# yhao-wang/DenseRetrievalToolkits

Hardware: AMD Instinct MI355X
Metric: queries/sec@top-1000, 10Mx768 corpus (BASELINE: passages encoded/sec + queries/sec@top-1000, 10Mx768 corpus, 1/2/4/8 GPU) (higher is better)
Workload: dtype bf16

## Files before the change

denseretrievaltoolkits_amd/_native.py:

```python
from __future__ import annotations

import ctypes
import os
import threading

import torch

from .build_native import LIB_PATH

DRT_OK = 0
DRT_EINVAL = -1
ROW_STATS_LEN = 34

_lock = threading.Lock()
_lib = None

c_i32 = ctypes.c_int32
c_i64 = ctypes.c_int64
c_sz = ctypes.c_size_t
c_vp = ctypes.c_void_p
c_f32 = ctypes.c_float
c_u64 = ctypes.c_uint64

_SIGNATURES = [
    ("drt_version", ctypes.c_char_p, []),
    ("drt_ip_topk_workspace", c_sz, [c_i64, c_i64, c_i32, c_i32]),
    ("drt_ip_topk_bf16", c_i32, [c_vp, c_i64, c_vp, c_i64, c_i32, c_i32, c_i64, c_vp, c_vp, c_vp, c_vp, c_sz, c_vp]),
    ("drt_ip_topk_resolve_workspace", c_sz, [c_i64, c_i64, c_i32]),
    ("drt_ip_topk_resolve", c_i32, [c_vp, c_i64, c_vp, c_i64, c_i32, c_i32, c_i64, c_vp, c_vp, c_vp, c_vp, c_sz,
                                    c_vp, c_vp]),
    ("drt_topk_merge", c_i32, [c_vp, c_vp, c_i64, c_i32, c_i32, c_i32, c_vp, c_vp, c_vp]),
    ("drt_ip_topk_sample_rank", c_i32, [c_i32]),
    ("drt_ip_topk_dist_workspace", c_sz, [c_i64, c_i64, c_i64, c_i32, c_i32]),
    ("drt_ip_topk_dist_sample", c_i32, [c_vp, c_i64, c_vp, c_i64, c_i64, c_i32, c_i32, c_vp, c_vp, c_sz, c_vp]),
    ("drt_ip_topk_dist_tau", c_i32, [c_vp, c_i64, c_i32, c_i32, c_vp, c_vp]),
    ("drt_ip_topk_dist_filter", c_i32, [c_vp, c_i64, c_vp, c_i64, c_i64, c_i32, c_i32, c_i64, c_vp, c_vp, c_vp,
                                        c_sz, c_vp]),
    ("drt_ip_topk_dist_filter_chunks", c_i32, [c_vp, c_i64, c_vp, c_i64, c_i64, c_i32, c_i32, c_i64, c_vp, c_vp,
                                               c_vp, c_i32, c_vp, c_sz, c_vp]),
    ("drt_ip_topk_tighten_rank", c_i32, [c_i64, c_i32, c_i32]),
    ("drt_ip_topk_filter_passes_workspace", c_sz, [c_i64, c_i64, c_i64, c_i32, c_i32]),
    ("drt_ip_topk_filter_passes", c_i32, [c_vp, c_i64, c_vp, c_i64, c_i64, c_i32, c_i32, c_i64, c_vp, c_vp,
                                          c_i32, c_i32, c_vp, c_vp, c_vp, c_sz, c_vp]),
    ("drt_ip_topk_dist_filter_lists", c_i32, [c_vp, c_i64, c_vp, c_i64, c_i64, c_i32, c_i32, c_i64, c_vp, c_i32,
                                              c_vp, c_vp, c_vp, c_sz, c_vp]),
    ("drt_ip_topk_dist_filter_lists_at", c_i32, [c_vp, c_i64, c_vp, c_i64, c_i64, c_i32, c_i32, c_i64, c_vp,
                                                 c_i32, c_i64, c_vp, c_vp, c_vp, c_sz, c_vp]),
    ("drt_topk_merge_packed", c_i32, [c_vp, c_i64, c_i32, c_i32, c_i64, c_vp, c_vp, c_vp, c_vp]),
    ("drt_topk_merge_packed_cert", c_i32, [c_vp, c_i64, c_i32, c_i32, c_i32, c_i64, c_vp, c_vp, c_vp, c_vp]),
    ("drt_topk_merge_packed_capped", c_i32, [c_vp, c_i64, c_i32, c_i32, c_i32, c_i32, c_i64, c_vp, c_vp, c_vp,
                                             c_vp]),
    ("drt_row_stats_bf16", c_i32, [c_vp, c_i64, c_i32, c_vp, c_i32, c_vp]),
    ("drt_refine_width", c_i32, [c_i32]),
    ("drt_ip_topk_exact_bf16", c_i32, [c_vp, c_i64, c_vp, c_i64, c_i32, c_i32, c_i64, c_vp, c_vp, c_vp, c_vp, c_vp,
                                       c_sz, c_vp]),
    ("drt_hit_metrics_i8", c_i32, [c_vp, c_i64, c_i64, c_vp, c_i32, c_vp, c_vp]),
    ("drt_answer_match_i32", c_i32, [c_vp, c_i32, c_vp, c_vp, c_i64, c_i64, c_i64, c_vp, c_vp, c_i32, c_i32, c_vp,
                                     c_vp, c_vp]),
    ("drt_ip_topk_resolve_exact", c_i32, [c_vp, c_i64, c_vp, c_i64, c_i32, c_i32, c_i64, c_vp, c_vp, c_vp, c_vp,
                                          c_vp, c_sz, c_vp, c_vp]),
    ("drt_ip_topk_resolve_wide_workspace", c_sz, [c_i64, c_i32]),
    ("drt_ip_topk_resolve_wide", c_i32, [c_vp, c_i64, c_vp, c_i64, c_i32, c_i32, c_i64, c_vp, c_vp, c_vp, c_vp,
                                         c_vp, c_sz, c_vp, c_vp]),
    ("drt_ip_topk_large_workspace", c_sz, [c_i32, c_i32]),
    ("drt_ip_topk_large", c_i32, [c_vp, c_i64, c_vp, c_i64, c_i32, c_i32, c_i64, c_vp, c_vp, c_vp, c_vp, c_vp, c_vp,
                                  c_sz, c_vp]),
    ("drt_ip_topk_large_keys", c_i32, [c_vp, c_i64, c_vp, c_i64, c_i32, c_i32, c_i64, c_vp, c_vp, c_vp, c_vp, c_vp,
                                       c_vp, c_vp, c_sz, c_vp]),
    ("drt_merge_exact", c_i32, [c_vp, c_vp, c_i64, c_i32, c_i32, c_vp, c_vp, c_vp]),
    ("drt_refine_delta_bf16", c_i32, [c_vp, c_i64, c_i32, c_vp, c_i64, c_i64, c_vp, c_vp, c_i32, c_i32, c_vp, c_vp,
                                      c_vp, c_vp, c_vp, c_vp]),
    ("drt_refine_delta_local_bf16", c_i32, [c_vp, c_i64, c_i32, c_vp, c_i64, c_i64, c_vp, c_vp, c_i32, c_i32, c_vp,
                                            c_vp, c_vp, c_vp, c_vp, c_vp]),
    ("drt_refine_sort", c_i32, [c_vp, c_vp, c_vp, c_vp, c_i64, c_i32, c_i32, c_vp, c_vp, c_vp]),
    ("drt_topk_exclude", c_i32, [c_vp, c_vp, c_i64, c_i32, c_vp, c_vp, c_vp, c_i32, c_i32, c_vp, c_vp, c_vp, c_vp]),
    ("drt_pair_scores_bf16", c_i32, [c_vp, c_i64, c_vp, c_i64, c_i32, c_vp, c_vp, c_i64, c_vp, c_vp]),
    ("drt_gemm_nt_bf16_f32", c_i32, [c_vp, c_vp, c_vp, c_i64, c_i64, c_i32, c_i64, c_vp]),
    ("drt_embed_ln", c_i32, [c_vp, c_vp, c_i64, c_i64, c_vp, c_vp, c_vp, c_vp, c_vp, c_f32, c_i32, c_vp, c_vp]),
    ("drt_linear_bf16", c_i32, [c_vp, c_vp, c_vp, c_vp, c_vp, c_i64, c_i64, c_i64, c_i32, c_vp]),
    ("drt_linear_workspace", c_sz, [c_i64, c_i64, c_i64]),
    ("drt_linear_bf16_ws", c_i32, [c_vp, c_vp, c_vp, c_vp, c_vp, c_i64, c_i64, c_i64, c_i32, c_vp, c_sz, c_vp]),
    ("drt_linear_ln_bf16_ws", c_i32, [c_vp, c_vp, c_vp, c_vp, c_vp, c_vp, c_f32, c_vp, c_vp, c_i64, c_i64, c_i64,
                                      c_vp, c_sz, c_vp]),
    ("drt_layernorm_f32_bf16", c_i32, [c_vp, c_i64, c_i32, c_vp, c_vp, c_f32, c_vp, c_vp]),
    ("drt_attention_fwd_lse_bf16", c_i32, [c_vp, c_vp, c_vp, c_vp, c_i64, c_i64, c_i32, c_i32, c_f32, c_vp]),
    ("drt_layernorm_bwd_workspace", c_sz, [c_i64, c_i32]),
    ("drt_layernorm_bwd_drop_bf16", c_i32, [c_vp, c_vp, c_vp, c_f32, c_i64, c_i32, c_vp, c_vp, c_vp, c_f32, c_u64,
                                            c_u64, c_vp, c_vp, c_vp, c_sz, c_vp]),
    ("drt_layernorm_bwd_sum_bf16", c_i32, [c_vp, c_vp, c_vp, c_f32, c_i64, c_i32, c_vp, c_vp, c_vp, c_f32, c_u64,
                                           c_u64, c_vp, c_vp, c_vp, c_vp, c_sz, c_vp]),
    ("drt_linear_bf16_ex", c_i32, [c_vp, c_vp, c_vp, c_vp, c_vp, c_vp, c_vp, c_i64, c_i64, c_i64, c_i32, c_f32, c_u64,
                                   c_u64, c_vp, c_sz, c_vp]),
    ("drt_layernorm_bwd_bf16", c_i32, [c_vp, c_vp, c_vp, c_f32, c_i64, c_i32, c_vp, c_vp, c_vp, c_vp, c_vp, c_sz,
                                       c_vp]),
    ("drt_colsum_workspace", c_sz, [c_i64, c_i64]),
    ("drt_colsum_bf16", c_i32, [c_vp, c_i64, c_i64, c_vp, c_vp, c_sz, c_vp]),
    ("drt_colsum_f32", c_i32, [c_vp, c_i64, c_i64, c_vp, c_vp, c_sz, c_vp]),
    ("drt_linear_dgelu_bias_workspace", c_sz, [c_i64, c_i64, c_i64]),
    ("drt_linear_dgelu_bias_bf16", c_i32, [c_vp, c_vp, c_vp, c_vp, c_i64, c_i64, c_i64, c_vp, c_vp, c_sz, c_vp]),
    ("drt_gelu_bwd_bf16", c_i32, [c_vp, c_vp, c_i64, c_vp, c_vp]),
    ("drt_linear_wgrad_workspace", c_sz, [c_i64, c_i64, c_i64]),
    ("drt_linear_wgrad_bf16", c_i32, [c_vp, c_vp, c_vp, c_i64, c_i64, c_i64, c_vp, c_sz, c_vp]),
    ("drt_transpose_bf16", c_i32, [c_vp, c_i64, c_i64, c_vp, c_vp]),
    ("drt_transpose_bf16_ld", c_i32, [c_vp, c_i64, c_i64, c_vp, c_i64, c_vp]),
    ("drt_embed_ln_pre", c_i32, [c_vp, c_vp, c_i64, c_i64, c_vp, c_vp, c_vp, c_vp, c_vp, c_f32, c_i32, c_vp, c_vp,
                                 c_vp]),
    ("drt_gelu_bf16", c_i32, [c_vp, c_i64, c_vp, c_vp]),
    ("drt_embedding_bwd", c_i32, [c_vp, c_vp, c_vp, c_i64, c_i64, c_i32, c_i64, c_vp, c_vp, c_vp, c_vp]),
    ("drt_embedding_bwd_types", c_i32, [c_vp, c_vp, c_i32, c_vp, c_i64, c_i64, c_i32, c_i64, c_vp, c_vp, c_vp,
                                         c_vp]),
    ("drt_attention_train_fwd_bf16", c_i32, [c_vp, c_vp, c_vp, c_vp, c_i64, c_i64, c_i32, c_i32, c_f32, c_f32,
                                             ctypes.c_uint64, ctypes.c_uint64, c_vp]),
    ("drt_attention_train_bwd_bf16", c_i32, [c_vp, c_vp, c_vp, c_vp, c_vp, c_vp, c_i64, c_i64, c_i32, c_i32, c_f32,
                                             c_f32, ctypes.c_uint64, ctypes.c_uint64, c_vp]),
    ("drt_dropout_add_bf16", c_i32, [c_vp, c_vp, c_i64, c_f32, ctypes.c_uint64, ctypes.c_uint64, c_vp, c_vp]),
    ("drt_attention_train_fwd_bits_bf16", c_i32, [c_vp, c_vp, c_vp, c_vp, c_vp, c_i64, c_i64, c_i32, c_i32, c_f32,
                                                  c_f32, c_u64, c_u64, c_vp]),
    ("drt_attention_train_bwd_bits_bf16", c_i32, [c_vp, c_vp, c_vp, c_vp, c_vp, c_vp, c_vp, c_i64, c_i64, c_i32,
                                                  c_i32, c_f32, c_f32, c_u64, c_u64, c_vp]),
    ("drt_attention_train_bwd_bias_workspace", c_sz, [c_i64, c_i32, c_i32]),
    ("drt_attention_train_bwd_bias_bf16", c_i32, [c_vp, c_vp, c_vp, c_vp, c_vp, c_vp, c_vp, c_i64, c_i64, c_i32,
                                                  c_i32, c_f32, c_f32, c_u64, c_u64, c_vp, c_vp, c_sz, c_vp]),
    ("drt_attention_bwd_bf16", c_i32, [c_vp, c_vp, c_vp, c_vp, c_vp, c_vp, c_i64, c_i64, c_i32, c_i32, c_f32, c_vp]),
    ("drt_layernorm_bf16", c_i32, [c_vp, c_i64, c_i32, c_vp, c_vp, c_f32, c_vp, c_vp]),
    ("drt_attention_bf16", c_i32, [c_vp, c_vp, c_vp, c_i64, c_i64, c_i32, c_i32, c_f32, c_vp]),
    ("drt_pool_bf16", c_i32, [c_vp, c_vp, c_i64, c_i64, c_i32, c_i32, c_vp, c_vp, c_vp]),
# ... 62 lines not shown
```

denseretrievaltoolkits_amd/csrc/search.hip:

```cpp
#include <cmath>

#include "profile.h"
#include "search_internal.h"

namespace drt {

constexpr int kHitCap = 1024;
constexpr int kTopRL = 4;

__host__ __device__ __forceinline__ int pass_tiles(int ntiles, int npass, int pass) {
  return npass <= 1 ? ntiles : (pass < ntiles ? (ntiles - 1 - pass) / npass + 1 : 0);
}

__device__ __forceinline__ void glds16(const void* gsrc, uint32_t lds_addr) {
  uint32_t keep;
  asm volatile(
      "s_mov_b32 %0, m0\n\t"
      "s_mov_b32 m0, %2\n\t"
      "s_nop 0\n\t"
      "global_load_lds_dwordx4 %1, off\n\t"
      "s_mov_b32 m0, %0"
      : "=&s"(keep)
      : "v"(gsrc), "s"(lds_addr)
      : "memory");
}

__device__ __forceinline__ void glds16_nt(const void* gsrc, uint32_t lds_addr) {
  uint32_t keep;
  asm volatile(
      "s_mov_b32 %0, m0\n\t"
      "s_mov_b32 m0, %2\n\t"
      "s_nop 0\n\t"
      "global_load_lds_dwordx4 %1, off nt\n\t"
      "s_mov_b32 m0, %0"
      : "=&s"(keep)
      : "v"(gsrc), "s"(lds_addr)
      : "memory");
}

__device__ __forceinline__ uint32_t lds_addr_of(const void* p) {
  return (uint32_t)(uintptr_t)(const __attribute__((address_space(3))) char*)p;
}

template <int N>
__device__ __forceinline__ void wait_vmcnt() {
  asm volatile("s_waitcnt vmcnt(%0)" ::"n"(N) : "memory");
}

__device__ __forceinline__ void lds_barrier() {
  asm volatile("s_waitcnt lgkmcnt(0)" ::: "memory");
  __builtin_amdgcn_s_barrier();
}

__device__ __forceinline__ void push_hit(const ScanArgs& a, int q_local,
                                         int64_t q, uint64_t key, uint32_t* hit_n,
                                         uint64_t* hk, uint16_t* hq) {
  const uint32_t p = atomicAdd(hit_n, 1u);
  if (p < (uint32_t)kHitCap) {
    hk[p] = key;
    hq[p] = (uint16_t)q_local;
  } else {
    const uint32_t g = atomicAdd(a.counts + q * kCntStride, 1u);
    if (g < (uint64_t)a.cap) ((uint64_t*)a.out)[q * a.cap + g] = key;
  }
}

template <int NT>
__device__ __forceinline__ void flush_hits_agg(const ScanArgs& a, int64_t qbase, uint32_t n, const uint64_t* hk,
                                               const uint16_t* hq, uint32_t* qcnt, uint32_t* qoff) {
  n = n < (uint32_t)kHitCap ? n : (uint32_t)kHitCap;
  for (int i = threadIdx.x; i < kQueriesPerWG; i += NT) qcnt[i] = 0;
  lds_barrier();
  uint32_t rank[(kHitCap + NT - 1) / NT];
#pragma unroll
  for (int u = 0; u < (kHitCap + NT - 1) / NT; ++u) {
    const uint32_t i = threadIdx.x + u * NT;
    if (i < n) rank[u] = atomicAdd(&qcnt[hq[i]], 1u);
  }
  lds_barrier();
  for (int q = threadIdx.x; q < kQueriesPerWG; q += NT) {
    const uint32_t c = qcnt[q];
    qoff[q] = (c && qbase + q < a.nq) ? atomicAdd(a.counts + (qbase + q) * kCntStride, c) : 0u;
  }
  lds_barrier();
#pragma unroll
  for (int u = 0; u < (kHitCap + NT - 1) / NT; ++u) {
    const uint32_t i = threadIdx.x + u * NT;
    if (i < n) {
      const int ql = hq[i];
      const uint32_t g = qoff[ql] + rank[u];
      if (g < (uint64_t)a.cap) ((uint64_t*)a.out)[(qbase + ql) * a.cap + g] = hk[i];
    }
  }
}

// ... 314 lines not shown
  for (int64_t it = 0; it < my_tiles; ++it) {
    const int64_t tile = t0 + it * tstep;
    const int64_t younger = my_tiles - 1 - it;
    wait_tiles_younger<C::GLDS_PER_WAVE>((int)(younger < C::PD - 1 ? younger : C::PD - 1));
    lds_barrier();

    if (MODE == SCAN_FILTER) {
      const uint32_t n = *hit_n;
      if (n >= (uint32_t)(kHitCap / 2)) {
        if (AGG) flush_hits_agg<NW * 64>(a, qbase, n, hk, hq, qcnt, qoff);
        else flush_hits<NW * 64>(a, qbase, n, hk, hq);
        lds_barrier();
        if (tid == 0) *hit_n = 0;
        lds_barrier();
      }
    }
    if (it + C::PD < my_tiles)
      issue_tile16<D, NW>(a, ring + nslot * C::TILE_BYTES, tile + C::PD * tstep, wave, lane);

    const int64_t rowbase = tile * kT16 + 4 * kq;
    if ((it & 1) == 0) {
      mma_tile(accA, buf);
      if (it > 0) epilogue(accB, rbB);
      rbA = rowbase;
    } else {
      mma_tile(accB, buf);
      epilogue(accA, rbA);
      rbB = rowbase;
    }
    buf = (buf + 1 == C::NBUF) ? 0 : buf + 1;
    nslot = (nslot + 1 == C::NBUF) ? 0 : nslot + 1;
  }

  if (my_tiles & 1) epilogue(accA, rbA);
  else epilogue(accB, rbB);

  if (MODE == SCAN_TOPR) {
#pragma unroll
    for (int b = 0; b < QB; ++b) {
      if (!qok[b]) continue;
      uint32_t* o = (uint32_t*)a.out + qg[b] * a.cap + ((int64_t)blockIdx.x * 4 + kq) * kTopRL;
#pragma unroll
      for (int i = 0; i < kTopRL; ++i) o[i] = topl[b][i];
    }
  }
  if (MODE == SCAN_FILTER) {
    lds_barrier();
    const uint32_t nf = *hit_n;
    if (AGG) flush_hits_agg<NW * 64>(a, qbase, nf, hk, hq, qcnt, qoff);
    else flush_hits<NW * 64>(a, qbase, nf, hk, hq);
  }
}

constexpr int kWaveSeg = kHitCap / 8;

__device__ __forceinline__ void wave_flush_hits(const ScanArgs& a, int64_t qw, const uint64_t* hk,
                                                const uint8_t* hq, int n, int lane) {
  for (int i = lane; i < n; i += 64) {
    const uint64_t key = hk[i];
    const int64_t q = qw + hq[i];
    const uint32_t g = atomicAdd(a.counts + q * kCntStride, 1u);
    if (g < (uint64_t)a.cap) ((uint64_t*)a.out)[q * a.cap + g] = key;
  }
}

template <int D, bool NT = true>
__global__ __launch_bounds__(512, 1) void ip_scan16r_kernel(ScanArgs a) {
  constexpr int NW = 8;
  using C = Scan16Cfg<D, NW>;
  constexpr int PD = C::NBUF;
  __shared__ __attribute__((aligned(16))) char smem[C::LDS_BYTES];

  const int tid = threadIdx.x;
  const int wave = __builtin_amdgcn_readfirstlane(tid >> 6);
  const int lane = tid & 63;
  const int r = lane & 15;
  const int kq = lane >> 4;
  uint64_t* hk = (uint64_t*)(smem + C::HIT_KEY_OFF) + wave * kWaveSeg;
  uint8_t* hq = (uint8_t*)(smem + C::HIT_Q_OFF) + wave * kWaveSeg;

  const int64_t qbase = (int64_t)blockIdx.y * kQueriesPerWG;
  const int tmul = a.npass > 1 ? a.npass : 1;
  const int tph = a.npass > 1 ? a.pass : 0;
  const int tall = (int)((a.nrows + kT16 - 1) / kT16);
  const int ntiles = pass_tiles(tall, a.npass, a.pass);
  const uint32_t nrows = (uint32_t)a.nrows;
  const int t0 = blockIdx.x;
  const int tstep = gridDim.x;
  const int my_tiles = t0 < ntiles ? (ntiles - 1 - t0) / tstep + 1 : 0;
  if (my_tiles == 0) return;
  const int partial_tile = ((a.nrows & (kT16 - 1)) != 0 && (tall - 1) % tmul == tph) ? ntiles - 1 : -1;
  const uint32_t ring = lds_addr_of(smem);
  const int64_t tile_stride = (int64_t)tstep * tmul * kT16 * a.ldp * 2;
  const char* next_base = (const char*)(a.P + ((int64_t)t0 * tmul + tph) * kT16 * a.ldp);

  const int64_t qw = qbase + wave * 16;
  const int64_t qg = qw + r;
  const bool qok = qg < a.nq;
  const int64_t qs = qok ? qg : 0;
  bf16x8 qf[C::KS];
#pragma unroll
  for (int s = 0; s < C::KS; ++s) qf[s] = *(const bf16x8*)(a.Q + qs * a.ldq + s * 32 + kq * 8);
  float tau = __builtin_nanf("");
  {
    const float tv = a.tau[qs];
    tau = qok ? tv : tau;
  }
  if (!qok) {
#pragma unroll
    for (int s = 0; s < C::KS; ++s) qf[s] = (bf16x8){};
  }
#pragma unroll
  for (int s = 0; s < C::KS; ++s) asm volatile("" ::"v"(qf[s]));
  asm volatile("" ::"v"(tau));
  asm volatile("s_waitcnt vmcnt(0)" ::: "memory");

  LeanTile<D, NW> lt;
  lt.init(a, wave, lane);
#pragma unroll
  for (int p = 0; p < PD; ++p) {
    if (p < my_tiles) {
      const int tile = t0 + p * tstep;
      lt.template issue<NT>(a, ring + p * C::TILE_BYTES, next_base, tile == partial_tile, tile * tmul + tph, wave,
                            lane);
      next_base += tile_stride;
    }
  }
  if (wave >= NW / 2) __builtin_amdgcn_s_setprio(1);
  {
    const int last = my_tiles - 1 < PD - 1 ? my_tiles - 1 : PD - 1;
    wait_tiles_younger<C::GLDS_PER_WAVE>((int)last);
  }
  lds_barrier();

  const int sw = (r >> 1) & 7;
  int aoff[2];
#pragma unroll
  for (int m = 0; m < 2; ++m) aoff[m] = r * 128 + (((4 * m + kq) ^ sw) << 4);
  bf16x8 af[C::KS];
#pragma unroll
  for (int s = 0; s < C::KS; ++s) af[s] = *(const bf16x8*)(smem + (s >> 1) * (kT16 * 128) + aoff[s & 1]);

  auto mma_roll = [&](f32x4& acc, int nslot) {
    const char* nb = smem + nslot * C::TILE_BYTES;
    acc = (f32x4){0.f, 0.f, 0.f, 0.f};
#pragma unroll
    for (int s = 0; s < C::KS; ++s) {
      acc = __builtin_amdgcn_mfma_f32_16x16x32_bf16(af[s], qf[s], acc, 0, 0, 0);
      af[s] = *(const bf16x8*)(nb + (s >> 1) * (kT16 * 128) + aoff[s & 1]);
      __builtin_amdgcn_sched_barrier(0);
    }
  };
  int wcnt = 0;
  auto epilogue = [&](const f32x4& acc, uint32_t rowbase) {
    const float mx = fmaxf(fmaxf(acc[0], acc[1]), fmaxf(acc[2], acc[3])) - tau;
    if (__ballot(mx >= 0.0f) == 0ull) return;
    bool hv[4];
    uint64_t mv[4];
    int cv[4];
#pragma unroll
    for (int j = 0; j < 4; ++j) {
      hv[j] = acc[j] >= tau && rowbase + j < nrows;
      mv[j] = __ballot(hv[j]);
      cv[j] = __builtin_popcountll(mv[j]);
    }
    const int tot = cv[0] + cv[1] + cv[2] + cv[3];
    if (wcnt + tot <= kWaveSeg) {
      int base = wcnt;
#pragma unroll
      for (int j = 0; j < 4; ++j) {
        if (hv[j]) {
          const int pos = base + (int)__builtin_amdgcn_mbcnt_hi((uint32_t)(mv[j] >> 32),
                                                                __builtin_amdgcn_mbcnt_lo((uint32_t)mv[j], 0u));
          hk[pos] = ((uint64_t)desc_key(acc[j]) << 32) | (uint64_t)(a.row_base + rowbase + j);
          hq[pos] = (uint8_t)r;
        }
        base += cv[j];
      }
      wcnt = base;
      return;
    }
#pragma unroll
    for (int j = 0; j < 4; ++j) {
      const bool hit = acc[j] >= tau && rowbase + j < nrows;
      const uint64_t m = __ballot(hit);
      if (m == 0ull) continue;
      const int c = __builtin_popcountll(m);
      if (wcnt + c > kWaveSeg) {
        wave_flush_hits(a, qw, hk, hq, wcnt, lane);
        wcnt = 0;
      }
      if (hit) {
        const int pos = wcnt + (int)__builtin_amdgcn_mbcnt_hi((uint32_t)(m >> 32),
                                                              __builtin_amdgcn_mbcnt_lo((uint32_t)m, 0u));
        hk[pos] = ((uint64_t)desc_key(acc[j]) << 32) | (uint64_t)(a.row_base + rowbase + j);
        hq[pos] = (uint8_t)r;
      }
      wcnt += c;
    }
  };

  f32x4 accA, accB;
  uint32_t rbA = 0, rbB = 0;
  int buf = 0;
  auto iter = [&](int it, f32x4& acc, uint32_t& rb, const f32x4& prev, uint32_t rb_prev) {
    const int tile = t0 + it * tstep;
    if (it + PD <= my_tiles) {
      wait_vmcnt<C::GLDS_PER_WAVE * (PD - 2)>();
    } else if (it + 1 < my_tiles) {
      wait_tiles_younger<C::GLDS_PER_WAVE>(my_tiles - 1 - it - 1);
    }
    lds_barrier();
    if (it + PD < my_tiles) {
      const int ntile = tile + PD * tstep;
      lt.template issue<NT>(a, ring + buf * C::TILE_BYTES, next_base, ntile == partial_tile, ntile * tmul + tph,
                            wave, lane);
      next_base += tile_stride;
    }
    const int nslot = buf + 1 == C::NBUF ? 0 : buf + 1;
    mma_roll(acc, nslot);
    if (it > 0) epilogue(prev, rb_prev);
    rb = (uint32_t)(tile * tmul + tph) * kT16 + 4 * kq;
    buf = nslot;
  };
  for (int it = 0; it < my_tiles; it += 2) {
    iter(it, accA, rbA, accB, rbB);
    if (it + 1 < my_tiles) iter(it + 1, accB, rbB, accA, rbA);
  }
  if (my_tiles & 1) epilogue(accA, rbA);
  else epilogue(accB, rbB);
  if (wcnt) wave_flush_hits(a, qw, hk, hq, wcnt, lane);
}

template <int D>
struct Scan32Cfg {
  static constexpr int KS = D / 32;
  static constexpr int RD = KS % 2 == 0 ? 2 : 1;
  static constexpr int TILE_BYTES = kT16 * D * 2;
  static constexpr int HIT_BYTES = kHitCap * 9;
  static constexpr int NB_RAW = (160 * 1024 - HIT_BYTES) / TILE_BYTES;
  static constexpr int NB = NB_RAW > 6 ? 6 : NB_RAW;
  static constexpr int RING_BYTES = NB * TILE_BYTES;
  static constexpr int LDS_BYTES = RING_BYTES + HIT_BYTES;
  static_assert(NB >= 3, "ring too small");
  static_assert(LDS_BYTES <= 160 * 1024, "LDS budget");
};
constexpr int kQueriesPerWG32 = 256;

template <int D>
__global__ __launch_bounds__(512, 1) void ip_scan32r_kernel(ScanArgs a) {
  constexpr int NW = 8;
  using C = Scan16Cfg<D, NW>;
  using C32 = Scan32Cfg<D>;
  constexpr int NB = C32::NB;
  constexpr int PD = NB - 1;
  constexpr int KS = C32::KS;
  constexpr int RD = C32::RD;
  constexpr int kSeg = kHitCap / NW;
  __shared__ __attribute__((aligned(16))) char smem[C32::LDS_BYTES];

  const int tid = threadIdx.x;
  const int wave = __builtin_amdgcn_readfirstlane(tid >> 6);
  const int lane = tid & 63;
  const int r = lane & 15;
  const int kq = lane >> 4;
  uint64_t* hk = (uint64_t*)(smem + C32::RING_BYTES) + wave * kSeg;
  uint8_t* hq = (uint8_t*)(smem + C32::RING_BYTES + kHitCap * 8) + wave * kSeg;

  const int64_t qbase = (int64_t)blockIdx.y * kQueriesPerWG32;
  const int tmul = a.npass > 1 ? a.npass : 1;
  const int tph = a.npass > 1 ? a.pass : 0;
  const int tall = (int)((a.nrows + kT16 - 1) / kT16);
  const int ntiles = pass_tiles(tall, a.npass, a.pass);
  const uint32_t nrows = (uint32_t)a.nrows;
  const int t0 = blockIdx.x;
  const int tstep = gridDim.x;
  const int my_tiles = t0 < ntiles ? (ntiles - 1 - t0) / tstep + 1 : 0;
  if (my_tiles == 0) return;
  const int partial_tile = ((a.nrows & (kT16 - 1)) != 0 && (tall - 1) % tmul == tph) ? ntiles - 1 : -1;
  const uint32_t ring = lds_addr_of(smem);
  const int64_t tile_stride = (int64_t)tstep * tmul * kT16 * a.ldp * 2;
  const char* next_base = (const char*)(a.P + ((int64_t)t0 * tmul + tph) * kT16 * a.ldp);

  const int64_t qw = qbase + wave * 32;
  bf16x8 qf0[KS], qf1[KS];
  float tau0, tau1;
  {
    const int64_t g0 = qw + r, g1 = qw + 16 + r;
    const bool ok0 = g0 < a.nq, ok1 = g1 < a.nq;
    const int64_t s0 = ok0 ? g0 : 0, s1 = ok1 ? g1 : 0;
#pragma unroll
    for (int s = 0; s < KS; ++s) {
      qf0[s] = *(const bf16x8*)(a.Q + s0 * a.ldq + s * 32 + kq * 8);
      qf1[s] = *(const bf16x8*)(a.Q + s1 * a.ldq + s * 32 + kq * 8);
    }
    const float v0 = a.tau[s0], v1 = a.tau[s1];
    tau0 = ok0 ? v0 : __builtin_nanf("");
    tau1 = ok1 ? v1 : __builtin_nanf("");
    if (!ok0) {
#pragma unroll
      for (int s = 0; s < KS; ++s) qf0[s] = (bf16x8){};
    }
    if (!ok1) {
#pragma unroll
      for (int s = 0; s < KS; ++s) qf1[s] = (bf16x8){};
    }
  }
#pragma unroll
  for (int s = 0; s < KS; ++s) asm volatile("" ::"v"(qf0[s]), "v"(qf1[s]));
  asm volatile("" ::"v"(tau0), "v"(tau1));
  asm volatile("s_waitcnt vmcnt(0)" ::: "memory");

  LeanTile<D, NW> lt;
  lt.init(a, wave, lane);
#pragma unroll
  for (int p = 0; p < PD; ++p) {
    if (p < my_tiles) {
      const int tile = t0 + p * tstep;
      lt.template issue<false>(a, ring + p * C::TILE_BYTES, next_base, tile == partial_tile, tile * tmul + tph, wave,
                               lane);
      next_base += tile_stride;
    }
  }
  if (wave >= NW / 2) __builtin_amdgcn_s_setprio(1);
  {
    const int last = my_tiles - 1 < PD - 1 ? my_tiles - 1 : PD - 1;
    wait_tiles_younger<C::GLDS_PER_WAVE>((int)last);
  }
  lds_barrier();

  const int sw = (r >> 1) & 7;
  int aoff[2];
#pragma unroll
  for (int m = 0; m < 2; ++m) aoff[m] = r * 128 + (((4 * m + kq) ^ sw) << 4);
  auto frag = [&](int slot, int s) -> bf16x8 {
    return *(const bf16x8*)(smem + slot * C::TILE_BYTES + (s >> 1) * (kT16 * 128) + aoff[s & 1]);
  };
  bf16x8 af[RD];
#pragma unroll
  for (int s = 0; s < RD; ++s) af[s] = frag(0, s);

  int wcnt = 0;
  auto append = [&](const f32x4& acc, float tau, int ql, uint32_t rowbase) {
    const float mx = fmaxf(fmaxf(acc[0], acc[1]), fmaxf(acc[2], acc[3])) - tau;
    if (__ballot(mx >= 0.0f) == 0ull) return;
#pragma unroll
    for (int j = 0; j < 4; ++j) {
      const bool hit = acc[j] >= tau && rowbase + j < nrows;
      const uint64_t m = __ballot(hit);
      if (m == 0ull) continue;
      const int c = __builtin_popcountll(m);
      if (wcnt + c > kSeg) {
        wave_flush_hits(a, qw, hk, hq, wcnt, lane);
        wcnt = 0;
      }
      if (hit) {
        const int pos = wcnt + (int)__builtin_amdgcn_mbcnt_hi((uint32_t)(m >> 32),
                                                              __builtin_amdgcn_mbcnt_lo((uint32_t)m, 0u));
        hk[pos] = ((uint64_t)desc_key(acc[j]) << 32) | (uint64_t)(a.row_base + rowbase + j);
        hq[pos] = (uint8_t)ql;
      }
      wcnt += c;
    }
  };

  auto epilogue = [&](const f32x4& p0, const f32x4& p1, uint32_t rowbase) {
    append(p0, tau0, r, rowbase);
    append(p1, tau1, 16 + r, rowbase);
  };

  int buf = 0;
  auto iter = [&](int it, f32x4& acc0, f32x4& acc1, uint32_t& rb, const f32x4& prev0, const f32x4& prev1,
                  uint32_t rb_prev) {
    const int tile = t0 + it * tstep;
    if (it + PD <= my_tiles) {
      wait_vmcnt<C::GLDS_PER_WAVE * (PD - 2)>();
    } else if (it + 1 < my_tiles) {
      wait_tiles_younger<C::GLDS_PER_WAVE>(my_tiles - 1 - it - 1);
    }
    lds_barrier();
    const bool do_dma = it + PD < my_tiles;
    const int ntile = tile + PD * tstep;
    const int pslot = buf == 0 ? NB - 1 : buf - 1;
    const int nslot = buf + 1 == NB ? 0 : buf + 1;
    acc0 = (f32x4){0.f, 0.f, 0.f, 0.f};
    acc1 = (f32x4){0.f, 0.f, 0.f, 0.f};
#pragma unroll
    for (int s = 0; s < KS; ++s) {
      acc0 = __builtin_amdgcn_mfma_f32_16x16x32_bf16(af[s % RD], qf0[s], acc0, 0, 0, 0);
      acc1 = __builtin_amdgcn_mfma_f32_16x16x32_bf16(af[s % RD], qf1[s], acc1, 0, 0, 0);
      af[s % RD] = s + RD < KS ? frag(buf, s + RD) : frag(nslot, s + RD - KS);
      __builtin_amdgcn_sched_barrier(0);
      if (s == KS / 4 && do_dma) {
        lt.template issue<false>(a, ring + pslot * C::TILE_BYTES, next_base, ntile == partial_tile,
                                 ntile * tmul + tph, wave, lane);
        next_base += tile_stride;
      }
      __builtin_amdgcn_sched_barrier(0);
    }
    if (it > 0) epilogue(prev0, prev1, rb_prev);
    rb = (uint32_t)(tile * tmul + tph) * kT16 + 4 * kq;
    buf = nslot;
  };
  f32x4 a0, a1, b0, b1;
  uint32_t rbA = 0, rbB = 0;
  for (int it = 0; it < my_tiles; it += 2) {
    iter(it, a0, a1, rbA, b0, b1, rbB);
    if (it + 1 < my_tiles) iter(it + 1, b0, b1, rbB, a0, a1, rbA);
  }
  if (my_tiles & 1) epilogue(a0, a1, rbA);
  else epilogue(b0, b1, rbB);
  if (wcnt) wave_flush_hits(a, qw, hk, hq, wcnt, lane);
}

struct TopkPlan : PlanHead {
  int64_t n, k, nq, nq_pad;
  bool sample;
  int64_t cap;
  int64_t m;
  int64_t stride;
  int64_t r;
  int64_t nchunk;
  int64_t kc;
  size_t off_cs, off_ci, off_delta, off_rcnt, total;
};

static size_t plan_refine_tail(TopkPlan& p) {
  p.kc = refine_width(p.k);
  WsBump b{p.head_end};
  p.off_cs = b.take((size_t)p.nq_pad * p.kc * 4);
  p.off_ci = b.take((size_t)p.nq_pad * p.kc * 8);
  p.off_delta = b.take((size_t)p.nq_pad * p.kc * 4);
  p.off_rcnt = b.take((size_t)p.nq_pad * 8);
  return b.o;
}

static double poisson_tail_ge(double lam, int64_t r) {
  double logp = -lam + r * std::log(lam) - std::lgamma((double)r + 1.0);
  double p = std::exp(logp), s = 0.0;
  for (int64_t i = r; i < r + 2000; ++i) {
    s += p;
    p *= lam / (double)(i + 1);
    if (p < 1e-30 * s) break;
  }
  return s;
}


static TopkPlan make_plan(int64_t nq, int64_t n, int64_t k) {
  TopkPlan p{};
  p.n = n;
  p.k = k;
  p.nq = nq;
  p.nq_pad = (nq + kQueriesPerWG - 1) / kQueriesPerWG * kQueriesPerWG;
  const int64_t target = hit_target(k);
  p.cap = 4 * target;
  if (n <= p.cap) {
    p.sample = false;
    p.cap = align_up(std::max<int64_t>(n, 4), 4);
    p.m = 0;
    p.stride = 1;
    p.r = 0;
  } else {
    p.sample = true;
    int64_t r = 1;
    while (poisson_tail_ge((double)k * r / (double)target, r) > 1e-9 && r < 100000) ++r;
    p.r = r;
    int64_t m = (r * n + target - 1) / target;
    if (m > n) m = n;
    p.stride = std::max<int64_t>(1, n / m);
    const int64_t m_cap = std::max<int64_t>(1, kKthChunk / r) * kKthChunk;
    if (m > m_cap) m = m_cap;
    p.stride = std::max<int64_t>(1, n / m);
    p.m = (n - p.stride / 2 + p.stride - 1) / p.stride;
    if (p.m > m_cap) p.m = m_cap;
    if (p.m < r) p.m = std::min<int64_t>(n, r);
    p.nchunk = (p.m + kKthChunk - 1) / kKthChunk;
  }
  static_cast<PlanHead&>(p) = plan_head_layout(p.nq_pad, p.cap, p.sample ? 8 : 4, p.m, p.nchunk * p.r);
  p.total = plan_refine_tail(p);
  return p;
}

static TopkPlan make_dist_plan(int64_t nq, int64_t n_local, int64_t n_global, int64_t k) {
  const TopkPlan g = make_plan(nq, n_global, k);
  TopkPlan p{};
  p.n = n_local;
  p.k = k;
  p.nq = nq;
  p.nq_pad = g.nq_pad;
  const int64_t target = hit_target(k);
  p.cap = std::max<int64_t>(g.cap, 4 * target);
  p.sample = g.sample;
  p.r = g.sample ? g.r : 0;
  p.stride = 1;
  p.m = 0;
  p.nchunk = 0;
  if (p.sample && n_local > 0) {
    int64_t m = (p.r * n_local + target - 1) / target;
    if (m > n_local) m = n_local;
    const int64_t m_cap = std::max<int64_t>(1, kKthChunk / p.r) * kKthChunk;
    if (m > m_cap) m = m_cap;
    p.stride = std::max<int64_t>(1, n_local / m);
    p.m = (n_local - p.stride / 2 + p.stride - 1) / p.stride;
    if (p.m > m_cap) p.m = m_cap;
    p.nchunk = (p.m + kKthChunk - 1) / kKthChunk;
  }
  static_cast<PlanHead&>(p) = plan_head_layout(p.nq_pad, p.cap, 8, p.m, p.nchunk * p.r);
  p.total = p.head_end;
  return p;
}

static int64_t rows_exp_hits(const TopkPlan& p, int64_t rows, int64_t n_global) {
  return p.sample ? std::max<int64_t>(1, hit_target(p.k) * rows / std::max<int64_t>(1, n_global)) : rows;
}

static int64_t pass_exp_hits(const TopkPlan& p, int64_t npasses, int64_t n_global) {
  return p.sample ? std::max<int64_t>(1, hit_target(p.k) * p.n / npasses / std::max<int64_t>(1, n_global))
                  : std::max<int64_t>(1, p.n / npasses);
}

static int scan_grid_x(int64_t ntiles) {
  int dev = 0, cus = 256;
  if (hipGetDevice(&dev) == hipSuccess) {
    int v = 0;
    if (hipDeviceGetAttribute(&v, hipDeviceAttributeMultiprocessorCount, dev) == hipSuccess && v > 0)
      cus = v;
  }
  const int64_t g = std::min<int64_t>(ntiles, (int64_t)cus);
  return (int)std::max<int64_t>(g, 1);
}

static dim3 scan16_grid(int64_t nq, int64_t nrows, int qpw = kQueriesPerWG) {
  const unsigned gy = (unsigned)((nq + qpw - 1) / qpw);
  const int64_t ntiles = (nrows + kT16 - 1) / kT16;
  int gx = scan_grid_x(ntiles);
  if (gy > 1 && ntiles >= 8) {
    const int cus = scan_grid_x((int64_t)1 << 40);
    const int share = std::max(8, (cus / (int)gy) & ~7);
    gx = (int)std::min<int64_t>(ntiles, share);
  }
  return dim3(gx, gy);
}

template <int D>
static int launch_scan_d(const ScanArgs& a, int mode, hipStream_t s) {
  if (a.nq == 0 || a.nrows == 0) return DRT_OK;
  constexpr bool kLean = D <= 768;
  if (a.npass > 1 && (mode != SCAN_FILTER || !kLean || a.row0 != 0 || a.rstride != 1 || a.pass < 0 ||
                      a.pass >= a.npass))
    return DRT_EINVAL;
  const int64_t ntiles = pass_tiles((int)((a.nrows + kT16 - 1) / kT16), a.npass, a.pass);
  if (ntiles == 0) return DRT_OK;
  const dim3 grid = scan16_grid(a.nq, ntiles * kT16);
  const unsigned gy = grid.y;
  if (mode == SCAN_FILTER) {
    const double eh = a.exp_hits > 0 ? (double)a.exp_hits : (double)a.cap / 4.0;
    const bool dense_hits = eh * 256.0 / (double)a.nrows >= 0.35;
    bool lean = false;
    if constexpr (kLean) {
      lean = a.row0 == 0 && a.rstride == 1;
      if (lean) {
        if (gy > 1) {
          const dim3 grid32 = scan16_grid(a.nq, ntiles * kT16, kQueriesPerWG32);
          hipLaunchKernelGGL((ip_scan32r_kernel<D>), grid32, dim3(512), 0, s, a);
        } else {
          hipLaunchKernelGGL((ip_scan16r_kernel<D, true>), grid, dim3(512), 0, s, a);
        }
      }
    }
    if (!lean) {
      if (dense_hits) hipLaunchKernelGGL((ip_scan16_kernel<D, SCAN_FILTER, 8, true>), grid, dim3(512), 0, s, a);
      else hipLaunchKernelGGL((ip_scan16_kernel<D, SCAN_FILTER, 8, false>), grid, dim3(512), 0, s, a);
    }
  } else if (mode == SCAN_TOPR) {
    hipLaunchKernelGGL((ip_scan16_kernel<D, SCAN_TOPR>), grid, dim3(512), 0, s, a);
  } else {
    hipLaunchKernelGGL((ip_scan16_kernel<D, SCAN_DENSE>), grid, dim3(512), 0, s, a);
  }
  return hip_status(hipGetLastError());
}

static int launch_scan_impl(const ScanArgs& a, int d, int mode, hipStream_t s) {
  switch (d) {
    case 64: return launch_scan_d<64>(a, mode, s);
    case 128: return launch_scan_d<128>(a, mode, s);
    case 192: return launch_scan_d<192>(a, mode, s);
    case 256: return launch_scan_d<256>(a, mode, s);
    case 320: return launch_scan_d<320>(a, mode, s);
    case 384: return launch_scan_d<384>(a, mode, s);
    case 448: return launch_scan_d<448>(a, mode, s);
    case 512: return launch_scan_d<512>(a, mode, s);
    case 576: return launch_scan_d<576>(a, mode, s);
    case 640: return launch_scan_d<640>(a, mode, s);
    case 704: return launch_scan_d<704>(a, mode, s);
    case 768: return launch_scan_d<768>(a, mode, s);
    case 832: return launch_scan_d<832>(a, mode, s);
    case 896: return launch_scan_d<896>(a, mode, s);
    case 960: return launch_scan_d<960>(a, mode, s);
    case 1024: return launch_scan_d<1024>(a, mode, s);
    default: return DRT_EINVAL;
  }
}

int launch_scan(const ScanArgs& a, int d, int mode, hipStream_t s, int family) {
  const ProfPair pp = prof_begin(family, s);
  const int rc = launch_scan_impl(a, d, mode, s);
  prof_end(pp, s);
  return rc;
}

static bool valid_dist_dims(int64_t nq, int64_t n_local, int64_t n_global, int32_t d, int32_t k) {
  return nq >= 0 && n_local >= 0 && n_global >= n_local && d > 0 && d % 64 == 0 && d <= 1024 && k >= 1 &&
         k <= kSelMaxK && n_global < (int64_t)0xFFFFFFFFll;
}

}

using namespace drt;

extern "C" {

const char* drt_version(void) {
  return "drt-mi355x 0.3 (gfx950; packed top-k lists: entry k = valid count << 32 | flags)";
}

size_t drt_ip_topk_workspace(int64_t nq, int64_t n, int32_t d, int32_t k) {
  if (!valid_dims(nq, n, d, k)) return 0;
  return make_plan(nq, n, k).total;
}

static int ip_topk_impl(const void* Q, int64_t nq, const void* P, int64_t n, int32_t d, int32_t k,
                        int64_t id_offset, float* out_scores, int64_t* out_ids, int32_t* status, void* ws,
                        size_t ws_bytes, const float* stats, hipStream_t s) {
  DRT_REQUIRE(valid_dims(nq, n, d, k));
  if (nq == 0) return DRT_OK;
  DRT_REQUIRE(Q && out_scores && out_ids && ws);
  const TopkPlan p = make_plan(nq, n, k);
  DRT_REQUIRE(ws_bytes >= p.total);
  char* w = (char*)ws;
  float* tau = (float*)(w + p.off_tau);
  uint32_t* cnt = (uint32_t*)(w + p.off_cnt);
  const bool refine = stats != nullptr && n > 0;

  SelectArgs sa{};
  sa.k = k;
  sa.nq = nq;
// ... 291 lines not shown
};

static int filter_setup(FilterRun& f, const void* Q, int64_t nq, const void* P, int64_t n_local, int64_t n_global,
                        int32_t d, int32_t k, int64_t id_offset, const void* thr, uint64_t* packed, void* ws,
                        size_t ws_bytes, void* stream) {
  DRT_REQUIRE(valid_dist_dims(nq, n_local, n_global, d, k));
  DRT_REQUIRE(id_offset >= 0 && id_offset + n_local <= n_global);
  if (nq == 0) return DRT_OK;
  DRT_REQUIRE(Q && thr && packed && ws);
  f.p = make_dist_plan(nq, n_local, n_global, k);
  DRT_REQUIRE(ws_bytes >= f.p.total);
  f.s = (hipStream_t)stream;
  f.w = (char*)ws;
  f.cnt = (uint32_t*)(f.w + f.p.off_cnt);
  f.sel = SelectArgs{};
  f.sel.in = f.w + f.p.off_keys;
  f.sel.in_stride = f.p.cap;
  f.sel.k = k;
  f.sel.nq = nq;
  f.sel.id_offset = id_offset;
  f.sel.out_packed = packed;
  f.sel.global_tau = true;
  f.scan = filter_scan_args(Q, nq, P, d, n_local, nullptr, f.cnt, f.w + f.p.off_keys, f.p.cap);
  return DRT_OK;
}

static int filter_begin(const FilterRun& f, bool zero_counts) {
  DRT_REQUIRE(f.scan.P != nullptr);
  if (zero_counts) DRT_CHECK_HIP(hipMemsetAsync(f.cnt, 0, f.p.nq_pad * 4 * kCntStride, f.s));
  return DRT_OK;
}

static int filter_select(FilterRun& f) {
  if (f.p.n == 0) return launch_select(f.sel, SEL_DENSE32, SEL_TOPK, f.s);
  f.sel.counts = f.cnt;
  f.sel.cap = f.p.cap;
  f.sel.n_total = f.p.n;
  return launch_select(f.sel, SEL_KEYS64, SEL_TOPK, f.s);
}

int drt_ip_topk_dist_filter(const void* Q, int64_t nq, const void* P, int64_t n_local, int64_t n_global, int32_t d,
                            int32_t k, int64_t id_offset, const float* tau, uint64_t* packed, void* ws,
                            size_t ws_bytes, void* stream) {
  FilterRun f;
  int rc = filter_setup(f, Q, nq, P, n_local, n_global, d, k, id_offset, tau, packed, ws, ws_bytes, stream);
  if (rc || nq == 0) return rc;
  if (n_local > 0) {
    if ((rc = filter_begin(f, true))) return rc;
    ScanArgs a = f.scan;
    a.tau = tau;
    a.exp_hits = rows_exp_hits(f.p, n_local, n_global);
    if ((rc = launch_scan(a, d, SCAN_FILTER, f.s, PROF_SCAN))) return rc;
  }
  return filter_select(f);
}

int drt_ip_topk_dist_filter_chunks(const void* Q, int64_t nq, const void* P, int64_t n_local, int64_t n_global,
                                   int32_t d, int32_t k, int64_t id_offset, const float* tau, uint64_t* packed,
                                   const int64_t* starts, int32_t nchunks, void* ws, size_t ws_bytes, void* stream) {
  DRT_REQUIRE(d <= 768 && n_local < ((int64_t)1 << 32));
  DRT_REQUIRE(starts != nullptr && nchunks >= 1 && starts[0] == 0 && starts[nchunks] == n_local);
  for (int c = 0; c < nchunks; ++c) DRT_REQUIRE(starts[c] <= starts[c + 1]);
  FilterRun f;
  int rc = filter_setup(f, Q, nq, P, n_local, n_global, d, k, id_offset, tau, packed, ws, ws_bytes, stream);
  if (rc || nq == 0) return rc;
  if (n_local > 0) {
    if ((rc = filter_begin(f, true))) return rc;
    for (int c = 0; c < nchunks; ++c) {
      const int64_t r0 = starts[c], rows = starts[c + 1] - starts[c];
      if (rows == 0) continue;
      ScanArgs a = f.scan;
      a.P += r0 * d;
      a.nrows = rows;
      a.row_base = (uint32_t)r0;
      a.tau = tau;
      a.exp_hits = rows_exp_hits(f.p, rows, n_global);
      if ((rc = launch_scan(a, d, SCAN_FILTER, f.s, PROF_SCAN))) return rc;
    }
  }
  return filter_select(f);
}

int32_t drt_ip_topk_tighten_rank(int64_t n_local, int32_t npasses, int32_t k) {
  if (n_local <= 0 || npasses <= 1 || k < 1) return 0;
  const int64_t tall = (n_local + kT16 - 1) / kT16;
  const int64_t t0 = (tall + npasses - 1) / npasses;
  if (t0 >= tall) return 0;
  const double C = (double)tall / (double)t0;
  for (int64_t r = 1; r < ((int64_t)1 << 24); ++r) {
    const double sigma = std::sqrt(C * (C - 1.0) * (double)r + (C - 1.0) * (double)r);
    if (C * (double)r - 5.0 * sigma >= (double)k) return (int32_t)r;
  }
  return 0;
}

size_t drt_ip_topk_filter_passes_workspace(int64_t nq, int64_t n_local, int64_t n_global, int32_t d, int32_t k) {
  if (!valid_dist_dims(nq, n_local, n_global, d, k)) return 0;
  const TopkPlan p = make_dist_plan(nq, n_local, n_global, k);
  return passes_layout(p.total, p.nq_pad).total;
}

int drt_ip_topk_filter_passes(const void* Q, int64_t nq, const void* P, int64_t n_local, int64_t n_global,
                              int32_t d, int32_t k, int64_t id_offset, const float* tau, uint64_t* packed,
                              int32_t npasses, int32_t r, float* tau1_out, uint32_t* pass0_out, void* ws,
                              size_t ws_bytes, void* stream) {
  DRT_REQUIRE(d <= 768 && n_local < ((int64_t)1 << 32) && npasses >= 1 && npasses <= 1024);
  FilterRun f;
  int rc = filter_setup(f, Q, nq, P, n_local, n_global, d, k, id_offset, tau, packed, ws, ws_bytes, stream);
  if (rc || nq == 0) return rc;
  const PassesLayout pl = passes_layout(f.p.total, f.p.nq_pad);
  DRT_REQUIRE(ws_bytes >= pl.total);
  if (r < 0) r = drt_ip_topk_tighten_rank(n_local, npasses, k);
  const int tall = (int)((n_local + kT16 - 1) / kT16);
  const bool tighten = r > 0 && n_local > 0 && pass_tiles(tall, npasses, 0) < tall;
  if (!tighten) {
    if (tau1_out) DRT_CHECK_HIP(hipMemcpyAsync(tau1_out, tau, (size_t)nq * 4, hipMemcpyDeviceToDevice, f.s));
    if (pass0_out) DRT_CHECK_HIP(hipMemsetAsync(pass0_out, 0, (size_t)nq * 16, f.s));
  }
  float* tau1 = tau1_out ? tau1_out : (float*)(f.w + f.p.off_tau);
  uint32_t* pass0 = pass0_out ? pass0_out : (uint32_t*)(f.w + pl.off_pass0);
  if (n_local > 0) {
    if ((rc = filter_begin(f, true))) return rc;
    for (int ps = 0; ps < npasses; ++ps) {
      if (pass_tiles(tall, npasses, ps) == 0) continue;
      ScanArgs a = f.scan;
      a.npass = npasses;
      a.pass = ps;
      a.tau = (tighten && ps > 0) ? tau1 : tau;
      a.exp_hits = pass_exp_hits(f.p, npasses, n_global);
      if ((rc = launch_scan(a, d, SCAN_FILTER, f.s, PROF_SCAN))) return rc;
      if (tighten && ps == 0) {
        const ProfPair pp = prof_begin(PROF_SELECT, f.s);
        launch_tighten(nq, (const uint64_t*)f.scan.out, f.p.cap, f.cnt, tau, (int)r, tau1, pass0, f.s);
        prof_end(pp, f.s);
        DRT_CHECK_HIP(hipGetLastError());
      }
    }
  }
  f.sel.pass0 = tighten ? pass0 : nullptr;
  return filter_select(f);
}

int drt_ip_topk_dist_filter_lists(const void* Q, int64_t nq, const void* P, int64_t n_local, int64_t n_global,
                                  int32_t d, int32_t k, int64_t id_offset, const uint32_t* lists, int32_t nlists,
                                  float* tau_out, uint64_t* packed, void* ws, size_t ws_bytes, void* stream) {
  const int32_t r = drt_ip_topk_sample_rank(k);
  return drt_ip_topk_dist_filter_lists_at(Q, nq, P, n_local, n_global, d, k, id_offset, lists, nlists,
                                          r > 0 ? nq * r : 0, tau_out, packed, ws, ws_bytes, stream);
}

int drt_ip_topk_dist_filter_lists_at(const void* Q, int64_t nq, const void* P, int64_t n_local, int64_t n_global,
                                     int32_t d, int32_t k, int64_t id_offset, const uint32_t* lists, int32_t nlists,
                                     int64_t lists_stride, float* tau_out, uint64_t* packed, void* ws,
                                     size_t ws_bytes, void* stream) {
  const int32_t r = drt_ip_topk_sample_rank(k);
  DRT_REQUIRE(r > 0 && nlists >= 1 && (int64_t)nlists * r <= kKthChunk);
  DRT_REQUIRE(nlists == 1 || lists_stride >= nq * r);
  FilterRun f;
  int rc = filter_setup(f, Q, nq, P, n_local, n_global, d, k, id_offset, lists, packed, ws, ws_bytes, stream);
  if (rc || nq == 0) return rc;
  float* tau = tau_out ? tau_out : (float*)(f.w + f.p.off_tau);
  launch_kth_final(nq, lists, (int)nlists, (int)r, lists_stride, (int64_t)r, tau, nullptr,
                   n_local > 0 ? f.cnt : nullptr, (int)r, f.s);
  DRT_CHECK_HIP(hipGetLastError());
  if (n_local > 0) {
    if ((rc = filter_begin(f, false))) return rc;
    ScanArgs a = f.scan;
    a.tau = tau;
    a.exp_hits = rows_exp_hits(f.p, n_local, n_global);
    if ((rc = launch_scan(a, d, SCAN_FILTER, f.s, PROF_SCAN))) return rc;
  }
  return filter_select(f);
}

}
```

denseretrievaltoolkits_amd/csrc/search_internal.h:

```cpp
#pragma once

#include <algorithm>
#include <vector>

#include "drt_common.h"

#define DRT_INTERNAL __attribute__((visibility("hidden")))

namespace drt {

constexpr int kQueriesPerWG = 128;
constexpr int kCntStride = 32;
constexpr int kSelMaxK = 2048;
constexpr int kKthChunk = 4096;
constexpr int64_t kWideCap = 65536;

enum { SEL_KEYS64 = 0, SEL_DENSE32 = 1 };
enum { SEL_TOPK = 0, SEL_KTH = 1 };

struct SelectArgs {
  const void* in;
  int64_t in_stride;
  const uint32_t* counts;
  int64_t n_in;
  int64_t cap;
  int64_t n_total;
  int k;
  int64_t nq;
  float* out_scores;
  int64_t* out_ids;
  int64_t ldo;
  int64_t id_offset;
  int32_t* status;
  const int32_t* qmap;
  float* tau;
  uint64_t* out_packed;
  bool global_tau;
  int k_cert;
  const uint32_t* pass0;
};

DRT_INTERNAL int launch_select(const SelectArgs& a, int input, int output, hipStream_t s);
DRT_INTERNAL bool kth_rank_fits(int64_t m, int64_t r);
DRT_INTERNAL void launch_kth_rank(int64_t nq, const uint32_t* in, int64_t stride, int64_t n, int r, float* tau,
                                  uint32_t* zero, hipStream_t s);
DRT_INTERNAL void launch_kth_partial(int64_t nchunk, int64_t nq, const uint32_t* in, int64_t stride, int64_t n, int r,
                                     uint32_t* part, hipStream_t s);
DRT_INTERNAL void launch_kth_final(int64_t nq, const uint32_t* part, int nlists, int r, int64_t lstride,
                                   int64_t qstride, float* tau, uint32_t* best, uint32_t* zero, int len,
                                   hipStream_t s);
DRT_INTERNAL void launch_tighten(int64_t nq, const uint64_t* keys, int64_t cap, const uint32_t* counts,
                                 const float* tau0, int r, float* tau1, uint32_t* pass0, hipStream_t s);

enum { SCAN_FILTER = 0, SCAN_DENSE = 1, SCAN_TOPR = 2 };

struct ScanArgs {
  const __bf16* Q;
  int64_t nq;
  int64_t ldq;
  const __bf16* P;
  int64_t ldp;
  int64_t row0;
  int64_t nrows;
  int64_t rstride;
  const float* tau;
  uint32_t* counts;
  void* out;
  int64_t cap;
  int64_t exp_hits;
  uint32_t row_base;
  int32_t npass;
  int32_t pass;
};

static inline ScanArgs scan_args(const void* Q, int64_t nq, const void* P, int32_t d) {
  ScanArgs a{};
  a.Q = (const __bf16*)Q;
  a.nq = nq;
  a.ldq = d;
  a.P = (const __bf16*)P;
  a.ldp = d;
  a.row0 = 0;
  a.rstride = 1;
  return a;
}

static inline ScanArgs filter_scan_args(const void* Q, int64_t nq, const void* P, int32_t d, int64_t n,
                                        const float* tau, uint32_t* counts, void* out, int64_t cap) {
  ScanArgs a = scan_args(Q, nq, P, d);
  a.nrows = n;
  a.tau = tau;
  a.counts = counts;
  a.out = out;
  a.cap = cap;
  return a;
}

DRT_INTERNAL int launch_scan(const ScanArgs& a, int d, int mode, hipStream_t s, int family);

struct RefineArgs {
  const __bf16* Q;
  int64_t nq;
  int32_t d;
  const __bf16* P;
  int64_t n_local;
  int64_t row_offset;
  const float* cs;
  const int64_t* ci;
  int32_t kc, k;
  const float* stats;
  const float* tau;
  float* delta;
  int32_t* cnt;
  int32_t* status;
  const int32_t* qmap;
  bool set_status;
  int32_t slice;
  float* out_s;
  int64_t* out_i;
};

DRT_INTERNAL int launch_refine(RefineArgs& ra, hipStream_t s);
DRT_INTERNAL int flagged_queries(const int32_t* status, int64_t nq, int32_t mask, int32_t want, hipStream_t s,
                                 std::vector<int32_t>& out);
DRT_INTERNAL int gather_queries(const void* Q, int32_t d, const int32_t* idx, int64_t nb, void* qbuf, void* qmap,
                                hipStream_t s);

static inline size_t align_up(size_t x, size_t a) { return (x + a - 1) / a * a; }

static inline int64_t hit_target(int64_t k) { return std::max<int64_t>(4096, 4 * k); }

static inline int64_t refine_width(int64_t k) {
  return std::min<int64_t>(kSelMaxK, k + std::max<int64_t>(256, k / 4));
}

static inline bool valid_dims(int64_t nq, int64_t n, int32_t d, int32_t k) {
  return nq >= 0 && n >= 0 && d > 0 && d % 64 == 0 && d <= 1024 && k >= 1 && k <= kSelMaxK &&
         n < (int64_t)0xFFFFFFFFll;
}


struct WsBump {
  size_t o = 0;
  size_t take(size_t bytes) {
    const size_t at = o;
    o = align_up(o + bytes, 256);
    return at;
  }
};

struct PlanHead {
  size_t off_tau, off_cnt, off_keys, off_sample, off_part, head_end;
};
static inline PlanHead plan_head_layout(int64_t nq_pad, int64_t cap, int key_bytes, int64_t m, int64_t part_keys) {
  WsBump b;
  PlanHead h;
  h.off_tau = b.take((size_t)nq_pad * 4);
  h.off_cnt = b.take((size_t)nq_pad * 4 * kCntStride);
  h.off_keys = b.take((size_t)nq_pad * cap * key_bytes);
  h.off_sample = b.take((size_t)nq_pad * align_up(m, 4) * 4);
  h.off_part = b.take((size_t)nq_pad * part_keys * 4);
  h.head_end = b.o;
  return h;
}

struct PassesLayout {
  size_t off_pass0, total;
};
static inline PassesLayout passes_layout(size_t plan_total, int64_t nq_pad) {
  WsBump b;
  b.take(plan_total);
  PassesLayout l;
  l.off_pass0 = b.take((size_t)nq_pad * 16);
  l.total = b.o;
  return l;
}

static inline int64_t resolve_width(int64_t n) { return align_up(std::max<int64_t>(n, 4), 4); }

struct ResolveLayout {
  size_t qbuf, scores, qmap, cand_s, cand_i, delta, cnt, total;
};
static inline ResolveLayout resolve_layout(int64_t chunk, int64_t n, int32_t d, int64_t kc = kSelMaxK) {
  WsBump b;
  ResolveLayout l;
  l.qbuf = b.take((size_t)chunk * d * 2);
  l.scores = b.take((size_t)chunk * resolve_width(n) * 4);
  l.qmap = b.take((size_t)chunk * 4);
  l.cand_s = b.take((size_t)chunk * kSelMaxK * 16 + chunk * 8);
  l.cand_i = l.cand_s + (size_t)chunk * kc * 4;
  l.delta = l.cand_s + (size_t)chunk * kc * 12;
  l.cnt = l.cand_s + (size_t)chunk * kc * 16;
  l.total = b.o;
  return l;
}

struct WideLayout {
  size_t qbuf, qmap, tau, counts, keys, ekeys, total;
};
static inline WideLayout wide_layout(int32_t d) {
  const size_t B = kQueriesPerWG;
  WsBump b;
  WideLayout l;
  l.qbuf = b.take(B * d * 2);
  l.qmap = b.take(B * 4);
  l.tau = b.take(B * 4);
  l.counts = b.take(B * kCntStride * 4);
  l.keys = b.take(B * kWideCap * 8);
  l.ekeys = b.take(B * kWideCap * 8);
  l.total = b.o;
  return l;
}

struct LargeLayout {
  WideLayout wide;
  size_t sel_k, sel_r, sel_n, bin_k, bin_r, total;
};
static inline LargeLayout large_layout(int32_t d, int32_t k) {
  const size_t B = kQueriesPerWG;
  LargeLayout l;
  l.wide = wide_layout(d);
  WsBump b{l.wide.total};
  l.sel_k = b.take(B * k * 8);
  l.sel_r = b.take(B * k * 4);
  l.sel_n = b.take(B * 4);
  l.bin_k = b.take(B * k * 8);
  l.bin_r = b.take(B * k * 4);
  l.total = b.o;
  return l;
}

}
```

denseretrievaltoolkits_amd/csrc/select.hip:

```cpp
#include "profile.h"
#include "search_internal.h"

namespace drt {

constexpr int kSelThreads = 512;
constexpr int kSelWaves = kSelThreads / 64;
constexpr int kSelBins = 1024;
constexpr int kSelBuf = 4096;
constexpr int kSelKPT = 16;
constexpr int kSelRegCap = kSelKPT * kSelThreads;

template <int INPUT>
__device__ __forceinline__ uint64_t sel_load(const SelectArgs& a, int64_t q, int64_t j) {
  if (INPUT == SEL_KEYS64) return ((const uint64_t*)a.in)[q * a.in_stride + j];
  const uint32_t v = ((const uint32_t*)a.in)[q * a.in_stride + j];
  return ((uint64_t)v << 32) | (uint64_t)(uint32_t)j;
}

__device__ __forceinline__ float key_score(uint64_t x) { return desc_key_to_score((uint32_t)(x >> 32)); }

__device__ __forceinline__ int score_bin(float s, float smin, float scale) {
  if (scale == 0.0f) return 0;
  return hist_bin((s - smin) * scale, kSelBins, __builtin_signbit(s) ? 0 : kSelBins - 1);
}
// ... 376 lines not shown
              cnt = bb[t];
              break;
            }
            run += bb[t];
          }
          const int64_t rem = kk - run;
          sh_prefix = prefix | ((uint64_t)d << shift);
          sh_mask = mask | (255ull << shift);
          sh_kk = rem;
          if ((int64_t)cnt == rem) sh_done = 1;
        }
      }
      __syncthreads();
    }
    const uint64_t thr = sh_prefix | ~sh_mask;
    if (tid == 0) sh_nsel = 0;
    __syncthreads();
    for (int64_t j = tid; j < c; j += kSelThreads) {
      const uint64_t x = sel_load<INPUT>(a, q, j);
      if (x <= thr) {
        const uint32_t p = atomicAdd(&sh_nsel, 1u);
        if (p < (uint32_t)kSelBuf) buf[p] = x;
      }
    }
    __syncthreads();
    nsel = (int)sh_nsel;
  }

  nsel = nsel < kSelBuf ? nsel : kSelBuf;
  int n2 = 1;
  while (n2 < nsel) n2 <<= 1;
  for (int i = nsel + tid; i < n2; i += kSelThreads) buf[i] = ~0ull;
  __syncthreads();
  block_bitonic(buf, n2);

  const int64_t orow = a.qmap ? (int64_t)a.qmap[q] : q;
  if (a.out_packed) {
    uint64_t* op = a.out_packed + orow * (int64_t)(a.k + 1);
    for (int j = tid; j < a.k; j += kSelThreads) {
      if (j < kk_total) {
        const uint64_t x = buf[j];
        op[j] = (x & 0xFFFFFFFF00000000ull) | (uint64_t)(uint32_t)(a.id_offset + (int64_t)(x & 0xFFFFFFFFull));
      } else {
        op[j] = ~0ull;
      }
    }
    if (tid == 0) {
      const uint64_t nval = (uint64_t)(kk_total < a.k ? kk_total : a.k);
      bool bad = INPUT == SEL_KEYS64 && c_raw > a.cap;
      if (INPUT == SEL_KEYS64 && a.pass0) {
        const uint32_t* t = a.pass0 + q * 4;
        if (t[2] && (int64_t)t[1] + (c_raw - (int64_t)t[0]) < (int64_t)a.k) bad = true;
      }
      op[a.k] = (nval << 32) | (bad ? 1ull : 0ull) | (c_raw > (int64_t)a.k ? 2ull : 0ull);
    }
    return;
  }
  float* os = a.out_scores + orow * a.ldo;
  int64_t* oi = a.out_ids + orow * a.ldo;
  for (int j = tid; j < a.k; j += kSelThreads) {
    if (j < kk_total) {
      const uint64_t x = buf[j];
      os[j] = key_score(x);
      oi[j] = a.id_offset + (int64_t)(x & 0xFFFFFFFFull);
    } else {
      os[j] = kPadScore;
      oi[j] = -1;
    }
  }
  if (a.status && tid == 0) {
    int st = 0;
    if (INPUT == SEL_KEYS64) {
      if (c_raw > a.cap) st = 1;
      const int64_t kq = a.k_cert > 0 ? a.k_cert : a.k;
      if (!a.global_tau && c_raw < kq && c_raw < a.n_total) st = 1;
    }
    a.status[orow] = st;
  }
}

constexpr int kTightThreads = 256;

__global__ __launch_bounds__(kTightThreads) void tighten_kernel(const uint64_t* keys, int64_t cap,
                                                                const uint32_t* counts, const float* tau0, int r,
                                                                float* tau1, uint32_t* pass0) {
  __shared__ uint32_t hist[256];
  __shared__ uint32_t sh_prefix, sh_rem;
  __shared__ uint32_t red[kTightThreads / 64];
  const int tid = threadIdx.x;
  const int64_t q = blockIdx.x;
  const uint32_t c = counts[q * kCntStride];
  const float t0 = tau0[q];
  if (!((int64_t)c <= cap && c >= (uint32_t)r && t0 == t0)) {
    if (tid == 0) {
      tau1[q] = t0;
      pass0[q * 4 + 0] = c;
      pass0[q * 4 + 1] = c;
      pass0[q * 4 + 2] = 0;
      pass0[q * 4 + 3] = 0;
    }
    return;
  }
  const uint64_t* kq = keys + q * cap;
  uint32_t prefix = 0, mask = 0, rem = (uint32_t)r;
  for (int shift = 24; shift >= 0; shift -= 8) {
    hist[tid] = 0;
    __syncthreads();
    for (uint32_t j = tid; j < c; j += kTightThreads) {
      const uint32_t key = (uint32_t)(kq[j] >> 32);
      if ((key & mask) == prefix) atomicAdd(&hist[(key >> shift) & 255], 1u);
    }
    __syncthreads();
    if (tid < 64) {
      const uint32_t bb[4] = {hist[4 * tid], hist[4 * tid + 1], hist[4 * tid + 2], hist[4 * tid + 3]};
      const uint32_t s4 = bb[0] + bb[1] + bb[2] + bb[3];
      uint32_t incl = s4;
#pragma unroll
      for (int o = 1; o < 64; o <<= 1) {
        const uint32_t v = __shfl_up(incl, o, 64);
        if (tid >= o) incl += v;
      }
      uint32_t run = incl - s4;
      if (run < rem && rem <= incl) {
        int dgt = 4 * tid;
#pragma unroll
        for (int t = 0; t < 3; ++t) {
          if (dgt == 4 * tid + t && run + bb[t] < rem) {
            run += bb[t];
            ++dgt;
          }
        }
        sh_prefix = prefix | ((uint32_t)dgt << shift);
        sh_rem = rem - run;
      }
    }
    __syncthreads();
    prefix = sh_prefix;
    rem = sh_rem;
    mask |= 255u << shift;
  }
  const float t1 = desc_key_to_score(prefix);
  uint32_t n = 0;
  for (uint32_t j = tid; j < c; j += kTightThreads) n += key_score(kq[j]) >= t1 ? 1u : 0u;
#pragma unroll
  for (int o = 32; o > 0; o >>= 1) n += __shfl_xor(n, o, 64);
  if ((tid & 63) == 0) red[tid >> 6] = n;
  __syncthreads();
  if (tid == 0) {
    uint32_t tot = 0;
    for (int w = 0; w < kTightThreads / 64; ++w) tot += red[w];
    tau1[q] = t1;
    pass0[q * 4 + 0] = c;
    pass0[q * 4 + 1] = tot;
    pass0[q * 4 + 2] = t1 > t0 ? 1u : 0u;
    pass0[q * 4 + 3] = 0;
  }
}

constexpr int kKthThreads = 512;

__device__ __forceinline__ void block_bitonic_u32(uint32_t* buf, int n2) { block_sort<uint32_t, kKthThreads>(buf, n2); }

constexpr int kKthPer = kKthChunk / kKthThreads;
constexpr int kKthBins = 256;
constexpr int kKthSel = 1024;

__global__ __launch_bounds__(kKthThreads) void kth_partial_kernel(const uint32_t* in, int64_t stride, int64_t n,
                                                                  int r, uint32_t* part) {
  __shared__ __attribute__((aligned(16))) uint32_t buf[kKthChunk];
  __shared__ uint32_t hist[kKthThreads / 64][kKthBins];
  __shared__ float red[2][kKthThreads / 64];
  __shared__ uint32_t sh_n;
  __shared__ int sh_bin;
  const int tid = threadIdx.x, wave = tid >> 6, lane = tid & 63;
  const int64_t q = blockIdx.y;
  const int nchunk = gridDim.x;
  const int64_t j0 = (int64_t)blockIdx.x * kKthChunk;
  const int cnt = (int)(n - j0 < kKthChunk ? n - j0 : kKthChunk);
  const uint32_t* src = in + q * stride + j0;

  uint32_t key[kKthPer];
#pragma unroll
  for (int v = 0; v < 2; ++v) {
    const int base = v * (kKthChunk / 2) + 4 * tid;
    if (base + 3 < cnt) {
      const u32x4 x = *(const u32x4*)(src + base);
#pragma unroll
      for (int u = 0; u < 4; ++u) key[4 * v + u] = x[u];
    } else {
#pragma unroll
      for (int u = 0; u < 4; ++u) key[4 * v + u] = base + u < cnt ? src[base + u] : 0xFFFFFFFFu;
    }
  }
  float hi = -__builtin_inff(), lo = __builtin_inff();
#pragma unroll
  for (int e = 0; e < kKthPer; ++e) {
    if (key[e] != 0xFFFFFFFFu) {
      const float sc = desc_key_to_score(key[e]);
      hi = fmaxf(hi, sc);
      lo = fminf(lo, sc);
    }
  }
#pragma unroll
  for (int o = 32; o > 0; o >>= 1) {
    hi = fmaxf(hi, __shfl_xor(hi, o, 64));
    lo = fminf(lo, __shfl_xor(lo, o, 64));
  }
  if (lane == 0) {
    red[0][wave] = hi;
    red[1][wave] = lo;
  }
  for (int i = tid; i < (kKthThreads / 64) * kKthBins; i += kKthThreads) (&hist[0][0])[i] = 0;
  __syncthreads();
#pragma unroll
  for (int w = 0; w < kKthThreads / 64; ++w) {
    hi = fmaxf(hi, red[0][w]);
    lo = fminf(lo, red[1][w]);
  }
  const float range = hi - lo;
  const float scale = hist_scale((float)kKthBins, range);
  int bins[kKthPer];
#pragma unroll
  for (int e = 0; e < kKthPer; ++e) {
    int bb = kKthBins;
    if (key[e] != 0xFFFFFFFFu) {
      const float sc = desc_key_to_score(key[e]);
      bb = scale == 0.0f ? 0 : hist_bin((hi - sc) * scale, kKthBins, __builtin_signbit(sc) ? kKthBins - 1 : 0);
      atomicAdd(&hist[wave][bb], 1u);
    }
    bins[e] = bb;
  }
  __syncthreads();
  if (tid < 64) {
    uint32_t c4[4];
    uint32_t s4 = 0;
#pragma unroll
    for (int t = 0; t < 4; ++t) {
// ... 197 lines not shown
  if (nsel <= kRankBuf) {
    int n2 = 1;
    while (n2 < nsel) n2 <<= 1;
    for (int i = nsel + tid; i < n2; i += kRankThreads) buf[i] = kPad;
    __syncthreads();
    block_sort<uint32_t, kRankThreads>(buf, n2);
    kth = r <= nsel ? buf[r - 1] : kPad;
  } else {
    if (tid == 0) {
      sh_rem = (uint32_t)r;
      sh_prefix = 0;
    }
    uint32_t mask = 0;
    for (int shift = 24; shift >= 0; shift -= 8) {
      if (tid < 256) hist[tid] = 0;
      __syncthreads();
      const uint32_t prefix = sh_prefix;
#pragma unroll
      for (int e = 0; e < kRankPer; ++e)
        if (key[e] <= T && (key[e] & mask) == prefix)
          atomicAdd(&hist[(key[e] >> shift) & 255u], 1u);
      __syncthreads();
      if (tid == 0) {
        uint32_t rem = sh_rem, dgt = 255;
        for (uint32_t dd = 0; dd < 256; ++dd) {
          if (hist[dd] >= rem) {
            dgt = dd;
            break;
          }
          rem -= hist[dd];
        }
        sh_rem = rem;
        sh_prefix = prefix | (dgt << shift);
      }
      mask |= 255u << shift;
      __syncthreads();
    }
    kth = sh_prefix;
  }
  if (tau && tid == 0) tau[q] = (kth == kPad) ? -__builtin_inff() : desc_key_to_score(kth);
}

int launch_select(const SelectArgs& a, int input, int output, hipStream_t s) {
  if (a.nq == 0) return DRT_OK;
  dim3 grid((unsigned)a.nq);
  const ProfPair pp = prof_begin(PROF_SELECT, s);
  struct End { const ProfPair& p; hipStream_t s; ~End() { prof_end(p, s); } } end_{pp, s};
  if (input == SEL_KEYS64 && output == SEL_TOPK)
    hipLaunchKernelGGL((select_kernel<SEL_KEYS64, SEL_TOPK>), grid, dim3(kSelThreads), 0, s, a);
  else if (input == SEL_DENSE32 && output == SEL_TOPK)
    hipLaunchKernelGGL((select_kernel<SEL_DENSE32, SEL_TOPK>), grid, dim3(kSelThreads), 0, s, a);
  else if (input == SEL_DENSE32 && output == SEL_KTH)
    hipLaunchKernelGGL((select_kernel<SEL_DENSE32, SEL_KTH>), grid, dim3(kSelThreads), 0, s, a);
  else
    return DRT_EINVAL;
  return hip_status(hipGetLastError());
}

bool kth_rank_fits(int64_t m, int64_t r) { return m <= kRankMaxKeys && r <= kRankBuf; }

void launch_kth_rank(int64_t nq, const uint32_t* in, int64_t stride, int64_t n, int r, float* tau, uint32_t* zero,
                     hipStream_t s) {
  const dim3 grid((unsigned)nq), block(kRankThreads);
  if (n <= (int64_t)kRankThreads * 8)
    hipLaunchKernelGGL(kth_rank_kernel<8>, grid, block, 0, s, in, stride, n, r, tau, zero);
  else if (n <= (int64_t)kRankThreads * 24)
    hipLaunchKernelGGL(kth_rank_kernel<24>, grid, block, 0, s, in, stride, n, r, tau, zero);
  else
    hipLaunchKernelGGL(kth_rank_kernel<kRankPerMax>, grid, block, 0, s, in, stride, n, r, tau, zero);
}

void launch_kth_partial(int64_t nchunk, int64_t nq, const uint32_t* in, int64_t stride, int64_t n, int r,
                        uint32_t* part, hipStream_t s) {
  hipLaunchKernelGGL(kth_partial_kernel, dim3((unsigned)nchunk, (unsigned)nq), dim3(kKthThreads), 0, s, in, stride, n,
                     r, part);
}

void launch_kth_final(int64_t nq, const uint32_t* part, int nlists, int r, int64_t lstride, int64_t qstride,
                      float* tau, uint32_t* best, uint32_t* zero, int len, hipStream_t s) {
  hipLaunchKernelGGL(kth_final_kernel, dim3((unsigned)nq), dim3(kKthThreads), 0, s, part, nlists, r, lstride, qstride,
                     tau, best, zero, len);
}

void launch_tighten(int64_t nq, const uint64_t* keys, int64_t cap, const uint32_t* counts, const float* tau0, int r,
                    float* tau1, uint32_t* pass0, hipStream_t s) {
  hipLaunchKernelGGL(tighten_kernel, dim3((unsigned)nq), dim3(kTightThreads), 0, s, keys, cap, counts, tau0, r, tau1,
                     pass0);
}

}
```

denseretrievaltoolkits_amd/csrc/torch_ops.cpp:

```cpp
#include <vector>

#include <torch/library.h>
#include <ATen/ATen.h>
#include <c10/core/DeviceGuard.h>
#include <ATen/hip/impl/HIPStreamMasqueradingAsCUDA.h>

#include "drt.h"

namespace {

using at::Tensor;

void* stream_of(const Tensor& t) {
  return (void*)at::hip::getCurrentHIPStreamMasqueradingAsCUDA(t.device().index()).stream();
}

void check_rc(int rc, const char* what) {
  TORCH_CHECK_VALUE(rc != DRT_EINVAL, what, ": invalid argument (DRT_EINVAL)");
  TORCH_CHECK(rc == DRT_OK, what, ": HIP error ", rc);
}

void need_gpu(const Tensor& t, const char* name) {
  TORCH_CHECK(t.is_cuda(), "drt ops run on the GPU only (", name, " is on ", t.device(),
              "; no CPU fallback exists)");
// ... 302 lines not shown
  check_rc(drt_ip_topk_dist_tau((const uint32_t*)lists.data_ptr<int32_t>(), lists.size(1), (int32_t)lists.size(0),
                                (int32_t)k, tau.data_ptr<float>(), stream_of(lists)),
           "drt_ip_topk_dist_tau");
  return tau;
}

struct FilterPrelude {
  c10::OptionalDeviceGuard guard;
  Tensor q, p, thr, ws;
  size_t wsb = 0;
  int64_t n_global, k;

  FilterPrelude(const Tensor& q_, const Tensor& p_, const Tensor& thr_, bool thr_is_lists, const Tensor& packed,
                int64_t n_global_, int64_t k_, bool passes_ws = false)
      : n_global(n_global_), k(k_) {
    need(q_, "q", at::kBFloat16, 2);
    need(p_, "p", at::kBFloat16, 2);
    if (thr_is_lists) need(thr_, "lists", at::kInt, 3);
    else need(thr_, "tau", at::kFloat, 1);
    need(packed, "packed", at::kLong, 2);
    guard.reset_device(q_.device());
    q = q_.contiguous();
    p = p_.contiguous();
    thr = thr_is_lists ? thr_ : thr_.contiguous();
    TORCH_CHECK_VALUE(thr_is_lists || thr.size(0) == q.size(0), "tau must hold one threshold per query");
    TORCH_CHECK_VALUE(packed.is_contiguous() && packed.size(0) == q.size(0) && packed.size(1) == k + 1,
                      "packed must be a contiguous [nq, k + 1] tensor");
    ws = dist_ws(q, p.size(0), n_global, k, &wsb, passes_ws);
  }
  template <class Fn, class... Mid>
  void call(Fn fn, const char* what, int64_t id_offset, Mid... mid) const {
    check_rc(fn(q.data_ptr(), q.size(0), p.size(0) ? p.data_ptr() : nullptr, p.size(0), n_global, (int32_t)q.size(1),
                (int32_t)k, id_offset, mid..., ws.data_ptr(), wsb, stream_of(q)),
             what);
  }
};

void dist_filter_into(const Tensor& q_, const Tensor& p_, int64_t n_global, int64_t k, int64_t id_offset,
                      const Tensor& tau_, Tensor& packed) {
  const FilterPrelude f(q_, p_, tau_, false, packed, n_global, k);
  f.call(drt_ip_topk_dist_filter, "drt_ip_topk_dist_filter", id_offset, f.thr.data_ptr<float>(),
         (uint64_t*)packed.data_ptr<int64_t>());
}

Tensor dist_filter(const Tensor& q, const Tensor& p, int64_t n_global, int64_t k, int64_t id_offset,
                   const Tensor& tau) {
  need(q, "q", at::kBFloat16, 2);
  Tensor packed = at::empty({q.size(0), k + 1}, q.options().dtype(at::kLong));
  dist_filter_into(q, p, n_global, k, id_offset, tau, packed);
  return packed;
}

void dist_filter_chunks_into(const Tensor& q_, const Tensor& p_, int64_t n_global, int64_t k, int64_t id_offset,
                             const Tensor& tau_, at::IntArrayRef starts, Tensor& packed) {
  const FilterPrelude f(q_, p_, tau_, false, packed, n_global, k);
  TORCH_CHECK_VALUE(starts.size() >= 2 && starts.front() == 0 && starts.back() == f.p.size(0),
                    "starts must run from 0 to the shard's row count");
  for (size_t c = 1; c < starts.size(); ++c) TORCH_CHECK_VALUE(starts[c - 1] <= starts[c], "starts must not decrease");
  TORCH_CHECK_VALUE(f.q.size(1) <= 768, "chunked filtering takes d <= 768");
  const std::vector<int64_t> st(starts.begin(), starts.end());
  f.call(drt_ip_topk_dist_filter_chunks, "drt_ip_topk_dist_filter_chunks", id_offset, f.thr.data_ptr<float>(),
         (uint64_t*)packed.data_ptr<int64_t>(), st.data(), (int32_t)st.size() - 1);
}

void filter_passes_into(const Tensor& q_, const Tensor& p_, int64_t n_global, int64_t k, int64_t id_offset,
                        const Tensor& tau_, int64_t npasses, int64_t r, Tensor& packed,
                        const c10::optional<Tensor>& tau1, const c10::optional<Tensor>& pass0) {
  const FilterPrelude f(q_, p_, tau_, false, packed, n_global, k, true);
  TORCH_CHECK_VALUE(f.q.size(1) <= 768, "interleaved filter passes take d <= 768");
  TORCH_CHECK_VALUE(npasses >= 1 && npasses <= 1024, "npasses must be in [1, 1024]");
  if (tau1.has_value()) {
    need(*tau1, "tau1", at::kFloat, 1);
    TORCH_CHECK_VALUE(tau1->is_contiguous() && tau1->size(0) == f.q.size(0), "tau1 must be a contiguous [nq] tensor");
  }
  if (pass0.has_value()) {
    need(*pass0, "pass0", at::kInt, 2);
    TORCH_CHECK_VALUE(pass0->is_contiguous() && pass0->size(0) == f.q.size(0) && pass0->size(1) == 4,
                      "pass0 must be a contiguous [nq, 4] tensor");
  }
  f.call(drt_ip_topk_filter_passes, "drt_ip_topk_filter_passes", id_offset, f.thr.data_ptr<float>(),
         (uint64_t*)packed.data_ptr<int64_t>(), (int32_t)npasses, (int32_t)r,
         tau1.has_value() ? tau1->data_ptr<float>() : nullptr,
         pass0.has_value() ? (uint32_t*)pass0->data_ptr<int32_t>() : nullptr);
}

void filter_lists_into(const Tensor& q_, const Tensor& p_, int64_t n_global, int64_t k, int64_t id_offset,
                       const Tensor& lists, int64_t q0, Tensor& packed, const char* what) {
  const FilterPrelude f(q_, p_, lists, true, packed, n_global, k);
  TORCH_CHECK_VALUE(lists.is_contiguous(), "lists must be a contiguous [nlists, NQ, r] tensor");
  TORCH_CHECK_VALUE(q0 >= 0 && q0 + f.q.size(0) <= lists.size(1), "query rows [", q0, ", ", q0 + f.q.size(0),
                    ") outside the lists' ", lists.size(1), " rows");
  const int64_t r = lists.size(2);
  TORCH_CHECK_VALUE(r == drt_ip_topk_sample_rank((int32_t)k), "lists hold ", r, " keys per query, k=", k, " needs ",
                    drt_ip_topk_sample_rank((int32_t)k));
  f.call(drt_ip_topk_dist_filter_lists_at, what, id_offset, (const uint32_t*)lists.data_ptr<int32_t>() + q0 * r,
         (int32_t)lists.size(0), lists.size(1) * r, (float*)nullptr, (uint64_t*)packed.data_ptr<int64_t>());
}

void dist_filter_lists_into(const Tensor& q, const Tensor& p, int64_t n_global, int64_t k, int64_t id_offset,
                            const Tensor& lists, int64_t q0, Tensor& packed) {
  filter_lists_into(q, p, n_global, k, id_offset, lists, q0, packed, "drt_ip_topk_dist_filter_lists_at");
}

Tensor dist_filter_lists(const Tensor& q, const Tensor& p, int64_t n_global, int64_t k, int64_t id_offset,
                         const Tensor& lists_) {
  need(q, "q", at::kBFloat16, 2);
  need(p, "p", at::kBFloat16, 2);
  need(lists_, "lists", at::kInt, 3);
  TORCH_CHECK_VALUE(lists_.size(1) == q.size(0), "lists must be [nlists, nq, r]");
  Tensor packed = at::empty({q.size(0), k + 1}, q.options().dtype(at::kLong));
  filter_lists_into(q, p, n_global, k, id_offset, lists_.contiguous(), 0, packed, "drt_ip_topk_dist_filter_lists");
  return packed;
}

std::tuple<Tensor, Tensor, Tensor> merge_packed(const Tensor& parts_, int64_t k, int64_t n_global, int64_t k_cert) {
  need(parts_, "parts", at::kLong, 3);
  TORCH_CHECK_VALUE(parts_.size(2) >= 2 && parts_.size(2) <= k + 1,
                    "merge_packed expects [nparts, nq, lcap + 1] lists with lcap <= k");
  const c10::DeviceGuard g(parts_.device());
  const Tensor parts = parts_.contiguous();
  const int64_t nq = parts.size(1), lcap = parts.size(2) - 1;
  Tensor s = at::empty({nq, k}, parts.options().dtype(at::kFloat));
  Tensor i = at::empty({nq, k}, parts.options().dtype(at::kLong));
  Tensor st = at::empty({nq}, parts.options().dtype(at::kInt));
  if (lcap < k) {
    check_rc(drt_topk_merge_packed_capped((const uint64_t*)parts.data_ptr<int64_t>(), nq, (int32_t)parts.size(0),
                                          (int32_t)lcap, (int32_t)k, (int32_t)(k_cert > 0 ? k_cert : k), n_global,
                                          s.data_ptr<float>(), i.data_ptr<int64_t>(), st.data_ptr<int32_t>(),
                                          stream_of(parts)),
             "drt_topk_merge_packed_capped");
    return {s, i, st};
  }
  check_rc(drt_topk_merge_packed_cert((const uint64_t*)parts.data_ptr<int64_t>(), nq, (int32_t)parts.size(0),
                                      (int32_t)k, (int32_t)(k_cert > 0 ? k_cert : k), n_global, s.data_ptr<float>(),
                                      i.data_ptr<int64_t>(), st.data_ptr<int32_t>(), stream_of(parts)),
           "drt_topk_merge_packed_cert");
  return {s, i, st};
}

std::tuple<Tensor, Tensor, Tensor> topk_exclude(const Tensor& scores_, const Tensor& ids_, const Tensor& excl_,
                                                const Tensor& excl_off_, const c10::optional<Tensor>& ceiling_,
                                                int64_t skip, int64_t k_out) {
  need(scores_, "scores", at::kFloat, 2);
  need(ids_, "ids", at::kLong, 2);
  need(excl_, "excl", at::kLong, 1);
  need(excl_off_, "excl_off", at::kLong, 1);
  TORCH_CHECK_VALUE(scores_.sizes() == ids_.sizes(), "topk_exclude: scores ", scores_.sizes(), " and ids ",
                    ids_.sizes(), " differ in shape");
  TORCH_CHECK_VALUE(ids_.device() == scores_.device() && excl_.device() == scores_.device() &&
                        excl_off_.device() == scores_.device(),
                    "topk_exclude: every tensor must be on the scores' device ", scores_.device());
  const int64_t nq = scores_.size(0), k_in = scores_.size(1);
  TORCH_CHECK_VALUE(excl_off_.numel() == nq + 1, "excl_off: expected ", nq + 1, " offsets (nq + 1), got ",
                    excl_off_.numel());
  TORCH_CHECK_VALUE(k_out >= 1 && skip >= 0 && skip <= 0x7FFFFFFF && k_out <= 0x7FFFFFFF,
                    "topk_exclude: unsupported skip=", skip, " k_out=", k_out, " (skip >= 0, k_out >= 1)");
  TORCH_CHECK_VALUE(k_in >= 1 && k_in <= 32768, "topk_exclude: unsupported list length k_in=", k_in,
                    " (1 <= k_in <= 32768)");
  const c10::DeviceGuard g(scores_.device());
  const Tensor scores = scores_.contiguous(), ids = ids_.contiguous(), excl = excl_.contiguous(),
               excl_off = excl_off_.contiguous();
  Tensor ceiling;
  if (ceiling_.has_value()) {
    need(*ceiling_, "ceiling", at::kFloat, 1);
    TORCH_CHECK_VALUE(ceiling_->device() == scores.device() && ceiling_->numel() == nq,
                      "ceiling: expected a float [", nq, "] tensor on ", scores.device());
// ... 188 lines not shown
  if (mask.has_value()) {
    TORCH_CHECK(mask->numel() == B * L, "attention: mask must be [B, L]");
    m = mask->to(at::kLong).contiguous();
  }
  Tensor ctx = at::empty({T, heads * hd}, qkv.options());
  check_rc(drt_attention_bf16(qkv.data_ptr(), m.has_value() ? m->data_ptr<int64_t>() : nullptr, ctx.data_ptr(), B, L,
                              (int32_t)heads, (int32_t)hd, (float)scale, stream_of(qkv)),
           "drt_attention_bf16");
  return ctx;
}

Tensor layernorm(const Tensor& x_, const Tensor& gamma, const Tensor& beta, double eps) {
  need_gpu(x_, "x");
  const c10::DeviceGuard g(x_.device());
  const Tensor x = x_.contiguous();
  const int64_t H = x.size(-1), M = x.numel() / H;
  Tensor out = at::empty(x.sizes(), x.options().dtype(at::kBFloat16));
  int rc;
  if (x.scalar_type() == at::kFloat)
    rc = drt_layernorm_f32_bf16(x.data_ptr<float>(), M, (int32_t)H, gamma.data_ptr<float>(), beta.data_ptr<float>(),
                                (float)eps, out.data_ptr(), stream_of(x));
  else {
    TORCH_CHECK(x.scalar_type() == at::kBFloat16, "layernorm: x must be float or bfloat16");
    rc = drt_layernorm_bf16(x.data_ptr(), M, (int32_t)H, gamma.data_ptr<float>(), beta.data_ptr<float>(), (float)eps,
                            out.data_ptr(), stream_of(x));
  }
  check_rc(rc, "drt_layernorm");
  return out;
}

Tensor pool(const Tensor& hidden_, const c10::optional<Tensor>& mask, int64_t mode) {
  need(hidden_, "hidden", at::kBFloat16, 3);
  const c10::DeviceGuard g(hidden_.device());
  const Tensor hidden = hidden_.contiguous();
  const int64_t B = hidden.size(0), L = hidden.size(1), H = hidden.size(2);
  c10::optional<Tensor> m;
  if (mask.has_value()) m = mask->to(at::kLong).contiguous();
  Tensor reps = at::empty({B, H}, hidden.options().dtype(at::kFloat));
  check_rc(drt_pool_bf16(hidden.data_ptr(), m.has_value() ? m->data_ptr<int64_t>() : nullptr, B, L, (int32_t)H,
                         (int32_t)mode, reps.data_ptr<float>(), nullptr, stream_of(hidden)),
           "drt_pool_bf16");
  return reps;
}

Tensor l2_normalize(const Tensor& x_) {
  need(x_, "x", at::kFloat, 2);
  const c10::DeviceGuard g(x_.device());
  Tensor x = x_.clone(at::MemoryFormat::Contiguous);
  check_rc(drt_l2_normalize_f32(x.data_ptr<float>(), x.size(0), (int32_t)x.size(1), nullptr, stream_of(x)),
           "drt_l2_normalize_f32");
  return x;
}

}

TORCH_LIBRARY(drt, m) {
  m.def("ip_topk(Tensor q, Tensor p, int k, int id_offset=0, Tensor? stats=None) -> (Tensor, Tensor, Tensor)");
  m.def("ip_topk.out(Tensor q, Tensor p, int k, int id_offset, Tensor? stats=None, *, Tensor(a!) scores, "
        "Tensor(b!) ids, Tensor(c!) status) -> ()");
  m.def("ip_topk_resolve(Tensor q, Tensor p, int k, int id_offset, Tensor(a!) scores, Tensor(b!) ids, "
        "Tensor(c!) status, Tensor? stats=None) -> int");
  m.def("ip_topk_resolve_wide(Tensor q, Tensor p, int k, int id_offset, Tensor(a!) scores, Tensor(b!) ids, "
        "Tensor(c!) status, Tensor stats) -> int");
  m.def("ip_topk_large(Tensor q, Tensor p, int k, int id_offset, Tensor stats, Tensor tau) -> (Tensor, Tensor, Tensor)");
  m.def("ip_topk_large_keys(Tensor q, Tensor p, int k, int id_offset, Tensor stats, Tensor tau) -> "
        "(Tensor, Tensor, Tensor, Tensor)");
  m.def("merge_exact(Tensor keys, Tensor ids, int k) -> (Tensor, Tensor)");
  m.def("row_stats(Tensor p, Tensor? prev=None) -> Tensor");
  m.def("refine_delta(Tensor q, Tensor p, int row_offset, Tensor cand_scores, Tensor cand_ids, int k, Tensor stats, "
        "Tensor? tau, Tensor(a!) status, bool local=False) -> (Tensor, Tensor)");
  m.def("refine_sort(Tensor cand_scores, Tensor cand_ids, Tensor delta, Tensor cnt, int k) -> (Tensor, Tensor)");
  m.def("topk_merge(Tensor scores, Tensor ids, int k_out) -> (Tensor, Tensor)");
  m.def("dist_sample(Tensor q, Tensor p, int n_global, int k) -> Tensor");
  m.def("dist_tau(Tensor lists, int k) -> Tensor");
  m.def("dist_filter(Tensor q, Tensor p, int n_global, int k, int id_offset, Tensor tau) -> Tensor");
  m.def("dist_filter_lists(Tensor q, Tensor p, int n_global, int k, int id_offset, Tensor lists) -> Tensor");
  m.def("dist_filter_lists_into(Tensor q, Tensor p, int n_global, int k, int id_offset, Tensor lists, int q0, "
        "Tensor(a!) packed) -> ()");
  m.def("dist_filter_into(Tensor q, Tensor p, int n_global, int k, int id_offset, Tensor tau, Tensor(a!) packed) -> ()");
  m.def("dist_filter_chunks_into(Tensor q, Tensor p, int n_global, int k, int id_offset, Tensor tau, int[] starts, "
        "Tensor(a!) packed) -> ()");
  m.def("filter_passes_into(Tensor q, Tensor p, int n_global, int k, int id_offset, Tensor tau, int npasses, int r, "
        "Tensor(a!) packed, Tensor(b!)? tau1=None, Tensor(c!)? pass0=None) -> ()");
  m.def("merge_packed(Tensor parts, int k, int n_global, int k_cert=-1) -> (Tensor, Tensor, Tensor)");
  m.def("topk_exclude(Tensor scores, Tensor ids, Tensor excl, Tensor excl_off, Tensor? ceiling, int skip, int k_out) -> "
        "(Tensor, Tensor, Tensor)");
  m.def("pair_scores(Tensor q, Tensor p, Tensor qidx, Tensor rows) -> Tensor");
  m.def("score_ce_fwd(Tensor q, Tensor p, int target_stride, float scale) -> (Tensor, Tensor, Tensor)");
  m.def("score_ce_bwd(Tensor grad, Tensor q, Tensor p, Tensor scores, Tensor lse, int target_stride, "
        "float scale) -> (Tensor, Tensor)");
  m.def("score_kd_fwd(Tensor q, Tensor p, Tensor teacher, int group, float temperature, float w_ce, float w_kd, "
        "float scale) -> (Tensor, Tensor, Tensor, Tensor)");
  m.def("score_kd_bwd(Tensor grad, Tensor q, Tensor p, Tensor teacher, Tensor scores, Tensor lse, Tensor aux, "
        "int group, float temperature, float w_ce, float w_kd, float scale) -> (Tensor, Tensor)");
  m.def("embed_ln(Tensor input_ids, Tensor? token_type_ids, Tensor word, Tensor pos, Tensor type, Tensor gamma, "
        "Tensor beta, float eps) -> Tensor");
  m.def("linear(Tensor x, Tensor w, Tensor? bias, Tensor? residual, bool gelu=False, bool fp32_out=False) -> Tensor");
  m.def("attention(Tensor qkv, Tensor? mask, int batch, int heads, float scale) -> Tensor");
  m.def("layernorm(Tensor x, Tensor gamma, Tensor beta, float eps) -> Tensor");
  m.def("pool(Tensor hidden, Tensor? mask, int mode) -> Tensor");
  m.def("l2_normalize(Tensor x) -> Tensor");
}

TORCH_LIBRARY_IMPL(drt, CUDA, m) {
  m.impl("ip_topk", &ip_topk);
  m.impl("ip_topk.out", &ip_topk_out);
  m.impl("dist_filter_chunks_into", &dist_filter_chunks_into);
  m.impl("filter_passes_into", &filter_passes_into);
  m.impl("ip_topk_resolve", &ip_topk_resolve);
  m.impl("ip_topk_resolve_wide", &ip_topk_resolve_wide);
  m.impl("ip_topk_large", &ip_topk_large);
  m.impl("ip_topk_large_keys", &ip_topk_large_keys);
  m.impl("merge_exact", &merge_exact);
  m.impl("row_stats", &row_stats);
  m.impl("refine_delta", &refine_delta);
  m.impl("refine_sort", &refine_sort);
  m.impl("topk_merge", &topk_merge);
  m.impl("dist_sample", &dist_sample);
  m.impl("dist_tau", &dist_tau);
  m.impl("dist_filter", &dist_filter);
  m.impl("dist_filter_lists", &dist_filter_lists);
  m.impl("dist_filter_lists_into", &dist_filter_lists_into);
  m.impl("dist_filter_into", &dist_filter_into);
  m.impl("merge_packed", &merge_packed);
  m.impl("topk_exclude", &topk_exclude);
  m.impl("pair_scores", &pair_scores);
  m.impl("score_ce_fwd", &score_ce_fwd);
  m.impl("score_ce_bwd", &score_ce_bwd);
  m.impl("score_kd_fwd", &score_kd_fwd);
  m.impl("score_kd_bwd", &score_kd_bwd);
  m.impl("embed_ln", &embed_ln);
  m.impl("linear", &linear);
  m.impl("attention", &attention);
  m.impl("layernorm", &layernorm);
  m.impl("pool", &pool);
  m.impl("l2_normalize", &l2_normalize);
}
```

denseretrievaltoolkits_amd/kernels.py:

```python
from __future__ import annotations

from typing import Optional, Tuple

import torch

from . import _native, ops


def _require_device(*ts: torch.Tensor) -> None:
    for t in ts:
        if not t.is_cuda:
            raise ValueError("DRT kernels run on the GPU only (got a CPU tensor; no CPU fallback exists)")


def ip_topk_workspace_bytes(nq: int, n: int, d: int, k: int) -> int:
    return int(_native.load().drt_ip_topk_workspace(nq, n, d, k))


def ip_topk(q: torch.Tensor, p: torch.Tensor, k: int, id_offset: int = 0, resolve: bool = True,
            out: Optional[Tuple[torch.Tensor, torch.Tensor]] = None,
            status: Optional[torch.Tensor] = None,
            stats: Optional[torch.Tensor] = None) -> Tuple[torch.Tensor, torch.Tensor, torch.Tensor]:
    drt = ops.load()
    _require_device(q, p)
# ... 172 lines not shown


def row_stats(p: torch.Tensor, prev: Optional[torch.Tensor] = None) -> torch.Tensor:
    _require_device(p)
    return ops.load().row_stats(p, prev)


def refine_width(k: int) -> int:
    w = int(_native.load().drt_refine_width(k))
    if w <= 0:
        raise ValueError(f"unsupported k={k}")
    return w


def refine(q: torch.Tensor, p: torch.Tensor, row_offset: int, cand_s: torch.Tensor, cand_i: torch.Tensor, k: int,
           stats: torch.Tensor, tau: Optional[torch.Tensor], status: torch.Tensor, all_reduce_sum=None):
    _require_device(q, p, cand_s, cand_i, stats, status)
    drt = ops.load()
    delta, cnt = drt.refine_delta(q, p, row_offset, cand_s, cand_i, k, stats, tau, status, all_reduce_sum is None)
    if all_reduce_sum is not None:
        all_reduce_sum(delta)
    return drt.refine_sort(cand_s, cand_i, delta, cnt, k)


def topk_merge(scores: torch.Tensor, ids: torch.Tensor, k_out: int) -> Tuple[torch.Tensor, torch.Tensor]:
    _require_device(scores, ids)
    if scores.dim() != 3 or scores.shape != ids.shape:
        raise ValueError("topk_merge expects [nparts, nq, k] scores and ids")
    return ops.load().topk_merge(scores.float(), ids.long(), k_out)


def sample_rank(k: int) -> int:
    r = int(_native.load().drt_ip_topk_sample_rank(k))
    if r <= 0:
        raise ValueError(f"unsupported k={k}")
    return r


def dist_sample(q: torch.Tensor, p: torch.Tensor, n_global: int, k: int) -> torch.Tensor:
    _require_device(q, p)
    return ops.load().dist_sample(q, p, n_global, k)


def dist_tau(lists: torch.Tensor, k: int) -> torch.Tensor:
    _require_device(lists)
    return ops.load().dist_tau(lists, k)


def dist_filter(q: torch.Tensor, p: torch.Tensor, n_global: int, k: int, id_offset: int,
                tau: torch.Tensor) -> torch.Tensor:
    _require_device(q, p, tau)
    return ops.load().dist_filter(q, p, n_global, k, id_offset, tau)


def dist_filter_lists(q: torch.Tensor, p: torch.Tensor, n_global: int, k: int, id_offset: int,
                      lists: torch.Tensor) -> torch.Tensor:
    _require_device(q, p, lists)
    return ops.load().dist_filter_lists(q, p, n_global, k, id_offset, lists)


def dist_filter_into(q: torch.Tensor, p: torch.Tensor, n_global: int, k: int, id_offset: int, tau: torch.Tensor,
                     packed: torch.Tensor) -> None:
    _require_device(q, p, tau, packed)
    ops.load().dist_filter_into(q, p, n_global, k, id_offset, tau, packed)


def dist_filter_chunks_into(q: torch.Tensor, p: torch.Tensor, n_global: int, k: int, id_offset: int,
                            tau: torch.Tensor, starts, packed: torch.Tensor) -> None:
    _require_device(q, p, tau, packed)
    ops.load().dist_filter_chunks_into(q, p, n_global, k, id_offset, tau, [int(x) for x in starts], packed)


def tighten_rank(n_local: int, npasses: int, k: int) -> int:
    return int(_native.load().drt_ip_topk_tighten_rank(n_local, npasses, k))


def filter_passes_into(q: torch.Tensor, p: torch.Tensor, n_global: int, k: int, id_offset: int, tau: torch.Tensor,
                       npasses: int, packed: torch.Tensor, r: int = -1, tau1: Optional[torch.Tensor] = None,
                       pass0: Optional[torch.Tensor] = None) -> None:
    _require_device(q, p, tau, packed)
    ops.load().filter_passes_into(q, p, n_global, k, id_offset, tau, npasses, r, packed, tau1, pass0)


def dist_filter_lists_into(q: torch.Tensor, p: torch.Tensor, n_global: int, k: int, id_offset: int,
                           lists: torch.Tensor, q0: int, packed: torch.Tensor) -> None:
    _require_device(q, p, lists, packed)
    ops.load().dist_filter_lists_into(q, p, n_global, k, id_offset, lists, q0, packed)


def merge_packed(parts: torch.Tensor, k: int, n_global: int, k_cert: int = -1):
    _require_device(parts)
    if parts.dim() != 3 or not 2 <= parts.shape[2] <= k + 1:
        raise ValueError("merge_packed expects [nparts, nq, lcap + 1] with lcap <= k")
    return ops.load().merge_packed(parts, k, n_global, k_cert)


def exchange_cap(kc: int, nparts: int) -> int:
    if nparts <= 1 or nparts > 8:
        return kc
    cap = -(-5 * kc // (4 * nparts)) + 32
    cap = -(-cap // 64) * 64
    return kc if cap * 10 >= kc * 9 else cap


def filtered_depth(k: int, skip: int, max_excluded: int) -> int:
    if k < 1 or skip < 0 or max_excluded < 0:
        raise ValueError(f"filtered search needs k >= 1, skip >= 0 (k={k}, skip={skip})")
    depth = skip + k + max_excluded
    if depth > MAX_K_LARGE:
        raise ValueError(f"filtered search depth skip + k + max exclusions = {skip} + {k} + {max_excluded} = {depth} "
                         f"exceeds the limit {MAX_K_LARGE} (MAX_K_LARGE)")
    return depth


def topk_exclude(scores: torch.Tensor, ids: torch.Tensor, excl: torch.Tensor, excl_off: torch.Tensor,
                 k_out: int, skip: int = 0,
                 ceiling: Optional[torch.Tensor] = None) -> Tuple[torch.Tensor, torch.Tensor, torch.Tensor]:
    _require_device(scores, ids, excl, excl_off)
    if ceiling is not None:
        _require_device(ceiling)
    if scores.dim() != 2 or scores.shape != ids.shape:
        raise ValueError("topk_exclude expects [nq, k_in] scores and ids")
    return ops.load().topk_exclude(scores, ids, excl, excl_off, ceiling, skip, k_out)


def pair_scores(q: torch.Tensor, p: torch.Tensor, qidx: torch.Tensor, rows: torch.Tensor) -> torch.Tensor:
    _require_device(q, p, qidx, rows)
    if q.dtype != torch.bfloat16 or p.dtype != torch.bfloat16:
        raise ValueError("pair_scores expects bf16 queries and corpus")
    return ops.load().pair_scores(q, p, qidx.to(torch.int32), rows.to(torch.int64))


def gemm_nt_f32(a: torch.Tensor, b: torch.Tensor, out: Optional[torch.Tensor] = None) -> torch.Tensor:
    lib = _native.load()
    _require_device(a, b)
    if a.dtype != torch.bfloat16 or b.dtype != torch.bfloat16:
        raise ValueError("gemm_nt_f32 expects bf16 operands")
    a = a.contiguous()
    b = b.contiguous()
    m, d = a.shape
    n = b.shape[0]
    if out is None:
        out = torch.empty((m, n), dtype=torch.float32, device=a.device)
    _native.check(lib.drt_gemm_nt_bf16_f32(a.data_ptr(), b.data_ptr(), out.data_ptr(), m, n, d, out.stride(0),
                                           _native.stream_ptr(a.device)), "drt_gemm_nt_bf16_f32")
    return out
```

denseretrievaltoolkits_amd/ops.py:

```python
from __future__ import annotations

import os
import threading

import torch

from . import _native
from ._native import ROW_STATS_LEN
from .build_native import OPS_LIB_PATH

_lock = threading.Lock()
_loaded = False


def load():
    global _loaded
    if _loaded:
        return torch.ops.drt
    with _lock:
        if _loaded:
            return torch.ops.drt
        _native.load()
        if not os.path.exists(OPS_LIB_PATH):
            raise RuntimeError(f"torch custom-op library not found at {OPS_LIB_PATH}; build it with "
# ... 10 lines not shown
    @lib.register_fake("drt::ip_topk")
    def _(q, p, k, id_offset=0, stats=None):
        nq = q.shape[0]
        return (q.new_empty((nq, k), dtype=torch.float32), q.new_empty((nq, k), dtype=torch.int64),
                q.new_empty((nq,), dtype=torch.int32))

    @lib.register_fake("drt::ip_topk.out")
    def _(q, p, k, id_offset, stats=None, *, scores, ids, status):
        return None

    @lib.register_fake("drt::ip_topk_resolve")
    def _(q, p, k, id_offset, scores, ids, status, stats=None):
        return torch.library.get_ctx().new_dynamic_size()

    @lib.register_fake("drt::ip_topk_resolve_wide")
    def _(q, p, k, id_offset, scores, ids, status, stats):
        return torch.library.get_ctx().new_dynamic_size()

    @lib.register_fake("drt::ip_topk_large")
    def _(q, p, k, id_offset, stats, tau):
        nq = q.shape[0]
        return (q.new_empty((nq, k), dtype=torch.float32), q.new_empty((nq, k), dtype=torch.int64),
                q.new_empty((nq,), dtype=torch.int32))

    @lib.register_fake("drt::ip_topk_large_keys")
    def _(q, p, k, id_offset, stats, tau):
        nq = q.shape[0]
        return (q.new_empty((nq, k), dtype=torch.float32), q.new_empty((nq, k), dtype=torch.int64),
                q.new_empty((nq,), dtype=torch.int32), q.new_empty((nq, k), dtype=torch.int64))

    @lib.register_fake("drt::merge_exact")
    def _(keys, ids, k):
        nq = keys.shape[1]
        return keys.new_empty((nq, k), dtype=torch.float32), ids.new_empty((nq, k))

    @lib.register_fake("drt::row_stats")
    def _(p, prev=None):
        return p.new_empty((ROW_STATS_LEN,), dtype=torch.float32)

    @lib.register_fake("drt::refine_delta")
    def _(q, p, row_offset, cand_scores, cand_ids, k, stats, tau, status, local=False):
        return cand_scores.new_empty(cand_scores.shape), cand_scores.new_empty((cand_scores.shape[0], 2),
                                                                                 dtype=torch.int32)

    @lib.register_fake("drt::refine_sort")
    def _(cand_scores, cand_ids, delta, cnt, k):
        nq = cand_scores.shape[0]
        return cand_scores.new_empty((nq, k)), cand_ids.new_empty((nq, k))

    @lib.register_fake("drt::topk_merge")
    def _(scores, ids, k_out):
        nq = scores.shape[1]
        return scores.new_empty((nq, k_out)), ids.new_empty((nq, k_out))

    @lib.register_fake("drt::dist_sample")
    def _(q, p, n_global, k):
        r = int(_native.load().drt_ip_topk_sample_rank(k))
        return q.new_empty((q.shape[0], r), dtype=torch.int32)

    @lib.register_fake("drt::dist_tau")
    def _(lists, k):
        return lists.new_empty((lists.shape[1],), dtype=torch.float32)

    @lib.register_fake("drt::dist_filter")
    def _(q, p, n_global, k, id_offset, tau):
        return q.new_empty((q.shape[0], k + 1), dtype=torch.int64)

    @lib.register_fake("drt::dist_filter_lists")
    def _(q, p, n_global, k, id_offset, lists):
        return q.new_empty((q.shape[0], k + 1), dtype=torch.int64)

    @lib.register_fake("drt::dist_filter_into")
    def _(q, p, n_global, k, id_offset, tau, packed):
        return None

    @lib.register_fake("drt::dist_filter_chunks_into")
    def _(q, p, n_global, k, id_offset, tau, starts, packed):
        return None

    @lib.register_fake("drt::filter_passes_into")
    def _(q, p, n_global, k, id_offset, tau, npasses, r, packed, tau1=None, pass0=None):
        return None

    @lib.register_fake("drt::dist_filter_lists_into")
    def _(q, p, n_global, k, id_offset, lists, q0, packed):
        return None

    @lib.register_fake("drt::merge_packed")
    def _(parts, k, n_global, k_cert=-1):
        nq = parts.shape[1]
        return (parts.new_empty((nq, k), dtype=torch.float32), parts.new_empty((nq, k), dtype=torch.int64),
                parts.new_empty((nq,), dtype=torch.int32))

    @lib.register_fake("drt::topk_exclude")
    def _(scores, ids, excl, excl_off, ceiling, skip, k_out):
        nq = scores.shape[0]
        return (scores.new_empty((nq, k_out), dtype=torch.float32), ids.new_empty((nq, k_out), dtype=torch.int64),
                scores.new_empty((nq,), dtype=torch.int32))

    @lib.register_fake("drt::pair_scores")
    def _(q, p, qidx, rows):
        return q.new_empty((rows.shape[0],), dtype=torch.float32)

    @lib.register_fake("drt::score_ce_fwd")
    def _(q, p, target_stride, scale):
        return q.new_empty(()), q.new_empty((q.shape[0], p.shape[0])), q.new_empty((q.shape[0],))

    @lib.register_fake("drt::score_ce_bwd")
    def _(grad, q, p, scores, lse, target_stride, scale):
        return q.new_empty(q.shape), p.new_empty(p.shape)

    @lib.register_fake("drt::score_kd_fwd")
    def _(q, p, teacher, group, temperature, w_ce, w_kd, scale):
        m = q.shape[0]
        return q.new_empty(()), q.new_empty((m, p.shape[0])), q.new_empty((m,)), q.new_empty((m, 2))

    @lib.register_fake("drt::score_kd_bwd")
    def _(grad, q, p, teacher, scores, lse, aux, group, temperature, w_ce, w_kd, scale):
        return q.new_empty(q.shape), p.new_empty(p.shape)

    @lib.register_fake("drt::embed_ln")
    def _(input_ids, token_type_ids, word, pos, type, gamma, beta, eps):
        return input_ids.new_empty(tuple(input_ids.shape) + (word.shape[1],), dtype=torch.bfloat16)

    @lib.register_fake("drt::linear")
    def _(x, w, bias, residual, gelu=False, fp32_out=False):
        return x.new_empty((x.shape[0], w.shape[0]), dtype=torch.float32 if fp32_out else torch.bfloat16)

    @lib.register_fake("drt::attention")
    def _(qkv, mask, batch, heads, scale):
        return qkv.new_empty((qkv.shape[0], qkv.shape[1] // 3))

    @lib.register_fake("drt::layernorm")
    def _(x, gamma, beta, eps):
        return x.new_empty(x.shape, dtype=torch.bfloat16)

    @lib.register_fake("drt::pool")
    def _(hidden, mask, mode):
        return hidden.new_empty((hidden.shape[0], hidden.shape[2]), dtype=torch.float32)

    @lib.register_fake("drt::l2_normalize")
    def _(x):
        return x.new_empty(x.shape)

    def setup_context(ctx, inputs, output):
        q, p, target_stride, scale = inputs
        _, scores, lse = output
        ctx.save_for_backward(q, p, scores, lse)
        ctx.target_stride = int(target_stride)
        ctx.scale = float(scale)
        ctx.mark_non_differentiable(scores, lse)

    def backward(ctx, g_loss, g_scores, g_lse):
        q, p, scores, lse = ctx.saved_tensors
        dq, dp = torch.ops.drt.score_ce_bwd(g_loss, q, p, scores, lse, ctx.target_stride, ctx.scale)
        return dq, dp, None, None

    lib.register_autograd("drt::score_ce_fwd", backward, setup_context=setup_context)

    def kd_setup_context(ctx, inputs, output):
        q, p, teacher, group, temperature, w_ce, w_kd, scale = inputs
        _, scores, lse, aux = output
        ctx.save_for_backward(q, p, teacher, scores, lse, aux)
        ctx.kd_args = (int(group), float(temperature), float(w_ce), float(w_kd), float(scale))
        ctx.mark_non_differentiable(scores, lse, aux)

# ... 7 lines not shown
```

denseretrievaltoolkits_amd/search.py:

```python
from __future__ import annotations

from typing import Optional, Tuple

import numpy as np
import torch

from . import _native, comm, kernels, shards


def _as_device_bf16(x, device) -> torch.Tensor:
    if isinstance(x, np.ndarray):
        x = torch.from_numpy(np.ascontiguousarray(x))
    if not isinstance(x, torch.Tensor):
        raise TypeError(f"expected np.ndarray or torch.Tensor, got {type(x)}")
    return x.detach().to(device=device, dtype=torch.bfloat16).contiguous()


def _stage_host(*ts: torch.Tensor):
    dev = ts[0].device
    hs = [torch.empty(t.shape, dtype=t.dtype, pin_memory=True) for t in ts]
    with torch.cuda.device(dev):
        stream = torch.cuda.current_stream(dev)
        for h, t in zip(hs, ts):
            h.copy_(t, non_blocking=True)
        ev = torch.cuda.Event()
        ev.record(stream)
    return hs, ev


def _stage_status(st: torch.Tensor):
    if not st.is_cuda:
        return st, None
    (h,), ev = _stage_host(st)
    return h, ev


def _status_failed(h: torch.Tensor, ev) -> int:
    if ev is not None:
        ev.synchronize()
    return int(((h & 1) != 0).sum().item())


def _order_uncertified(h: torch.Tensor) -> int:
    return int(((h & 2) != 0).sum().item())


EXACT_ORDER = True


class _HostResult:
    __slots__ = ("hs", "ev")

    def __init__(self, s: torch.Tensor, i: torch.Tensor):
        self.hs, self.ev = _stage_host(s, i)

    def get(self, s: torch.Tensor, i: torch.Tensor, redone: bool):
        if redone:
            return s.cpu().numpy(), i.cpu().numpy()
        self.ev.synchronize()
        return self.hs[0].numpy(), self.hs[1].numpy()


def _pipeline(batches, enqueue, finish):
    pend = None
    for j, q in enumerate(batches):
        cur = enqueue(j, q)
        if pend is not None:
            yield finish(pend)
        pend = cur
    if pend is not None:
        yield finish(pend)


GROUP_QUERIES = 2048
GROUP_MIN_ROWS = 500_000
GROUP_CHUNK_ROWS = 1_250_000
TIGHTEN_AFTER_FIRST_PASS = True


def group_chunks(nrows: int, chunk_rows: int = None, nch: int = None):
    chunk_rows = GROUP_CHUNK_ROWS if chunk_rows is None else chunk_rows
    if nch is None:
        if chunk_rows <= 0 or nrows <= chunk_rows:
            return [(0, nrows)]
        nch = -(-nrows // chunk_rows)
    if nch <= 1:
        return [(0, nrows)]
    per = -(-nrows // nch)
    return [(min(nrows, c * per), min(nrows, (c + 1) * per)) for c in range(nch)]


def _groups(batches, cap=None):
    cap = GROUP_QUERIES if cap is None else cap
    grp, n = [], 0
    for q in batches:
        if grp and n + q.shape[0] > cap:
            yield grp
            grp, n = [], 0
        grp.append(q)
        n += q.shape[0]
    if grp:
        yield grp


def _reserve_group_memory(local, k: int, n_global: int, chunks=None):
    key = (k, n_global, GROUP_QUERIES)
    if getattr(local, "_group_reserved", None) == key or local.ntotal == 0:
        return
    kc = kernels.refine_width(k)
    nq = GROUP_QUERIES
    ws = int(_native.load().drt_ip_topk_dist_workspace(nq, local.ntotal, n_global, local.dp, kc))
    nparts = max(1, len(chunks or [0]))
    lists = nq * (kc + 1) * 8 * (nparts + 1)
    outs = nq * kc * (4 + 8 + 4) + nq * k * (4 + 8) * 2
    need = ws + lists + outs + (64 << 20)
    with torch.cuda.device(local.device):
        blk = torch.empty(need, dtype=torch.uint8, device=local.device)
        del blk
    local._group_reserved = key


class _SideChannel:
    __slots__ = ("stream", "group")

    def __init__(self, stream, group):
        self.stream, self.group = stream, group

    def gather(self, t: torch.Tensor) -> torch.Tensor:
        return comm.all_gather_stacked(t, self.group)

    def all_reduce_sum(self, t: torch.Tensor) -> torch.Tensor:
        return comm.all_reduce_sum_(t, self.group)


def _gtau_enqueue_group(local, qs, k: int, n_global: int, offset: int, gather, to_host: bool = False,
                        stats=None, all_reduce_sum=None, id_shift: int = 0, chunks=None, world: int = 1,
                        side: _SideChannel = None):
    sizes = [q.shape[0] for q in qs]
    qg = qs[0] if len(qs) == 1 else torch.cat(qs)
    best = local.dist_sample(qg, n_global, k)
    lists = gather(best).contiguous()
    tau = kernels.dist_tau(lists, k)
    kc = kernels.refine_width(k) if stats is not None else k
    lc = kernels.exchange_cap(kc, world) if world > 1 and getattr(local, "exchange_capped", True) else kc
    if chunks is not None and len(chunks) > 1 and qg.shape[1] <= 768:
        lists = torch.empty((qg.shape[0], lc + 1), dtype=torch.int64, device=qg.device)
        if TIGHTEN_AFTER_FIRST_PASS and world == 1 and offset == 0 and n_global == local.rows.shape[0]:
            kernels.filter_passes_into(qg, local.rows, n_global, lc, offset, tau, len(chunks), lists)
        else:
            starts = [a for a, _ in chunks] + [chunks[-1][1]]
            kernels.dist_filter_chunks_into(qg, local.rows, n_global, lc, offset, tau, starts, lists)
    elif chunks is not None and len(chunks) > 1:
        lists = torch.empty((len(chunks), qg.shape[0], kc + 1), dtype=torch.int64, device=qg.device)
        for c, (a, b) in enumerate(chunks):
            kernels.dist_filter_into(qg, local.rows[a:b], n_global, kc, offset + a, tau, lists[c])
    else:
        lists = torch.empty((qg.shape[0], lc + 1), dtype=torch.int64, device=qg.device)
        kernels.dist_filter_into(qg, local.rows, n_global, lc, offset, tau, lists)

    def exchange(gather, all_reduce_sum):
        allp = gather(lists)
        if lists.dim() == 3:
            allp = allp.reshape(-1, qg.shape[0], kc + 1)
        s, i, st = kernels.merge_packed(allp, kc, n_global, k_cert=k)
        if stats is not None:
            s, i = kernels.refine(qg, local.rows, offset, s, i, k, stats, tau, st, all_reduce_sum)
        if id_shift:
            i = torch.where(i >= 0, i + id_shift, i)
        h, ev = _stage_status(st)
        host = _HostResult(s, i) if to_host else None
        return s, i, st, h, ev, host

    if side is None:
        return (qs, sizes) + exchange(gather, all_reduce_sum)
    compute = torch.cuda.current_stream(qg.device)
    scanned = torch.cuda.Event()
    scanned.record(compute)
    with torch.cuda.stream(side.stream):
        side.stream.wait_event(scanned)
        for t in (lists, qg, tau):
            t.record_stream(side.stream)
        s, i, st, h, ev, host = exchange(side.gather, side.all_reduce_sum)
    for t in (s, i, st):
        t.record_stream(compute)
    return qs, sizes, s, i, st, h, ev, host


def _gtau_finish_group(pend, redo, wide=None):
    qs, sizes, s, i, st, h, ev, host = pend
    if ev is not None:
        ev.synchronize()
    bad = (h & 1) != 0
    wid = (h & 3) == 2
    res, o, nredo, nunc = [], 0, 0, 0
    hs = hi = None
    for q, nb in zip(qs, sizes):
        nw = int(wid[o:o + nb].sum()) if not bool(bad[o:o + nb].any()) else 0
        if nw and wide is not None:
            nunc += nw - wide(q, s[o:o + nb], i[o:o + nb], st[o:o + nb])
            res.append((s[o:o + nb].cpu().numpy(), i[o:o + nb].cpu().numpy()) if host is not None
                       else (s[o:o + nb], i[o:o + nb]))
        elif bool(bad[o:o + nb].any()):
            rs, ri = redo(q)
            res.append((rs.cpu().numpy(), ri.cpu().numpy()) if host is not None else (rs, ri))
            nredo += 1
        elif host is not None:
            nunc += nw
            if hs is None:
                hs, hi = host.get(s, i, False)
            res.append((hs[o:o + nb], hi[o:o + nb]))
        else:
            nunc += nw
            res.append((s[o:o + nb], i[o:o + nb]))
        o += nb
    return res, nredo, nunc


def filtered_depth(k: int, skip: int, excl_off: torch.Tensor, ntotal: int, depth: Optional[int] = None) -> int:
    if excl_off.dim() != 1 or excl_off.numel() < 1:
        raise ValueError("excl_off must be a 1-d tensor of nq + 1 offsets")
    longest = int((excl_off[1:] - excl_off[:-1]).max().item()) if excl_off.numel() > 1 else 0
    need = kernels.filtered_depth(k, skip, max(0, longest))
    if depth is not None:
        if depth > kernels.MAX_K_LARGE:
            raise ValueError(f"filtered search depth {depth} exceeds the limit {kernels.MAX_K_LARGE} (MAX_K_LARGE)")
        need = max(need, int(depth))
    return max(1, min(need, int(ntotal)))


def _filtered_iter(index, batches, k: int, excl: torch.Tensor, excl_off: torch.Tensor, skip: int, ceiling,
# ... 514 lines not shown
```

include/drt.h:

```cpp
#ifndef DRT_H_
#define DRT_H_

#include <stddef.h>
#include <stdint.h>

#ifdef __cplusplus
extern "C" {
#endif

#define DRT_OK 0
#define DRT_EINVAL (-1)
#define DRT_ROW_STATS_LEN 34

const char* drt_version(void);

size_t drt_ip_topk_workspace(int64_t nq, int64_t n, int32_t d, int32_t k);
int drt_ip_topk_bf16(const void* Q, int64_t nq, const void* P, int64_t n, int32_t d,
                     int32_t k, int64_t id_offset, float* out_scores, int64_t* out_ids,
                     int32_t* status, void* workspace, size_t workspace_bytes,
                     void* stream);

size_t drt_ip_topk_resolve_workspace(int64_t n_failed, int64_t n, int32_t d);
int drt_ip_topk_resolve(const void* Q, int64_t nq, const void* P, int64_t n, int32_t d,
                        int32_t k, int64_t id_offset, float* out_scores, int64_t* out_ids,
                        int32_t* status, void* workspace, size_t workspace_bytes,
                        int64_t* n_resolved, void* stream);

int drt_row_stats_bf16(const void* P, int64_t n, int32_t d, float* stats, int32_t accumulate, void* stream);
int32_t drt_refine_width(int32_t k);
int drt_ip_topk_exact_bf16(const void* Q, int64_t nq, const void* P, int64_t n, int32_t d, int32_t k,
                           int64_t id_offset, const float* stats, float* out_scores, int64_t* out_ids,
                           int32_t* status, void* workspace, size_t workspace_bytes, void* stream);
int drt_ip_topk_resolve_exact(const void* Q, int64_t nq, const void* P, int64_t n, int32_t d, int32_t k,
                              int64_t id_offset, const float* stats, float* out_scores, int64_t* out_ids,
                              int32_t* status, void* workspace, size_t workspace_bytes, int64_t* n_resolved,
                              void* stream);
size_t drt_ip_topk_resolve_wide_workspace(int64_t n, int32_t d);
int drt_ip_topk_resolve_wide(const void* Q, int64_t nq, const void* P, int64_t n, int32_t d, int32_t k,
                             int64_t id_offset, const float* stats, float* out_scores, int64_t* out_ids,
                             int32_t* status, void* workspace, size_t workspace_bytes, int64_t* n_resolved,
                             void* stream);
size_t drt_ip_topk_large_workspace(int32_t d, int32_t k);
int drt_ip_topk_large(const void* Q, int64_t nq, const void* P, int64_t n, int32_t d, int32_t k, int64_t id_offset,
                      const float* stats, const float* tau, float* out_scores, int64_t* out_ids, int32_t* status,
                      void* workspace, size_t workspace_bytes, void* stream);
int drt_ip_topk_large_keys(const void* Q, int64_t nq, const void* P, int64_t n, int32_t d, int32_t k,
                           int64_t id_offset, const float* stats, const float* tau, float* out_scores,
                           int64_t* out_ids, uint64_t* out_keys, int32_t* status, void* workspace,
                           size_t workspace_bytes, void* stream);
int drt_merge_exact(const uint64_t* keys, const int64_t* ids, int64_t nq, int32_t nparts, int32_t k,
                    float* out_scores, int64_t* out_ids, void* stream);
int drt_refine_delta_bf16(const void* Q, int64_t nq, int32_t d, const void* P, int64_t n_local,
                          int64_t row_offset, const float* cand_s, const int64_t* cand_i, int32_t kc,
                          int32_t k, const float* stats, const float* tau, float* delta, int32_t* cnt,
                          int32_t* status, void* stream);
int drt_refine_delta_local_bf16(const void* Q, int64_t nq, int32_t d, const void* P, int64_t n_local,
                                int64_t row_offset, const float* cand_s, const int64_t* cand_i, int32_t kc,
                                int32_t k, const float* stats, const float* tau, float* delta, int32_t* cnt,
                                int32_t* status, void* stream);
int drt_refine_sort(const float* cand_s, const int64_t* cand_i, const float* delta, const int32_t* cnt,
                    int64_t nq, int32_t kc, int32_t k, float* out_scores, int64_t* out_ids, void* stream);

int drt_answer_match_i32(const int32_t* tok, int32_t W, const int64_t* rows, const int64_t* slot_of, int64_t n_rows,
                         int64_t B, int64_t k, const int32_t* ans, const int32_t* alen, int32_t A, int32_t n_max,
                         const uint8_t* every, int8_t* hit, void* stream);

int drt_hit_metrics_i8(const int8_t* hit, int64_t B, int64_t k, const int32_t* topk, int32_t T, double* acc,
                       void* stream);

int drt_topk_merge(const float* scores, const int64_t* ids, int64_t nq, int32_t nparts,
                   int32_t k_in, int32_t k_out, float* out_scores, int64_t* out_ids,
                   void* stream);

int drt_topk_exclude(const float* scores, const int64_t* ids, int64_t nq, int32_t k_in, const int64_t* excl,
                     const int64_t* excl_off, const float* ceiling, int32_t skip, int32_t k_out,
                     float* out_scores, int64_t* out_ids, int32_t* out_count, void* stream);
int drt_pair_scores_bf16(const void* Q, int64_t nq, const void* P, int64_t n, int32_t d, const int32_t* qidx,
                         const int64_t* rows, int64_t npairs, float* out, void* stream);

int32_t drt_ip_topk_sample_rank(int32_t k);
size_t drt_ip_topk_dist_workspace(int64_t nq, int64_t n_local, int64_t n_global, int32_t d,
                                  int32_t k);
int drt_ip_topk_dist_sample(const void* Q, int64_t nq, const void* P, int64_t n_local,
                            int64_t n_global, int32_t d, int32_t k, uint32_t* best, void* ws,
                            size_t ws_bytes, void* stream);
int drt_ip_topk_dist_tau(const uint32_t* lists, int64_t nq, int32_t nlists, int32_t k, float* tau,
                         void* stream);
int drt_ip_topk_dist_filter(const void* Q, int64_t nq, const void* P, int64_t n_local,
                            int64_t n_global, int32_t d, int32_t k, int64_t id_offset,
                            const float* tau, uint64_t* packed, void* ws, size_t ws_bytes,
                            void* stream);
int drt_ip_topk_dist_filter_chunks(const void* Q, int64_t nq, const void* P, int64_t n_local,
                                   int64_t n_global, int32_t d, int32_t k, int64_t id_offset,
                                   const float* tau, uint64_t* packed, const int64_t* starts,
                                   int32_t nchunks, void* ws, size_t ws_bytes, void* stream);
int32_t drt_ip_topk_tighten_rank(int64_t n_local, int32_t npasses, int32_t k);
size_t drt_ip_topk_filter_passes_workspace(int64_t nq, int64_t n_local, int64_t n_global, int32_t d,
                                           int32_t k);
int drt_ip_topk_filter_passes(const void* Q, int64_t nq, const void* P, int64_t n_local,
                              int64_t n_global, int32_t d, int32_t k, int64_t id_offset,
                              const float* tau, uint64_t* packed, int32_t npasses, int32_t r,
                              float* tau1_out, uint32_t* pass0_out, void* ws, size_t ws_bytes,
                              void* stream);
int drt_ip_topk_dist_filter_lists(const void* Q, int64_t nq, const void* P, int64_t n_local,
                                  int64_t n_global, int32_t d, int32_t k, int64_t id_offset,
                                  const uint32_t* lists, int32_t nlists, float* tau_out,
                                  uint64_t* packed, void* ws, size_t ws_bytes, void* stream);
int drt_ip_topk_dist_filter_lists_at(const void* Q, int64_t nq, const void* P, int64_t n_local,
                                     int64_t n_global, int32_t d, int32_t k, int64_t id_offset,
                                     const uint32_t* lists, int32_t nlists, int64_t lists_stride,
                                     float* tau_out, uint64_t* packed, void* ws, size_t ws_bytes,
                                     void* stream);
int drt_topk_merge_packed(const uint64_t* parts, int64_t nq, int32_t nparts, int32_t k,
                          int64_t n_global, float* out_scores, int64_t* out_ids, int32_t* status,
                          void* stream);
int drt_topk_merge_packed_capped(const uint64_t* parts, int64_t nq, int32_t nparts, int32_t lcap, int32_t k,
                                 int32_t k_cert, int64_t n_global, float* out_scores, int64_t* out_ids,
                                 int32_t* status, void* stream);
int drt_topk_merge_packed_cert(const uint64_t* parts, int64_t nq, int32_t nparts, int32_t k,
                               int32_t k_cert, int64_t n_global, float* out_scores, int64_t* out_ids,
                               int32_t* status, void* stream);
int drt_gemm_nt_bf16_f32(const void* A, const void* B, float* C, int64_t m, int64_t n,
                         int32_t d, int64_t ldc, void* stream);

int drt_embed_ln(const int64_t* ids, const int64_t* type_ids, int64_t B, int64_t L,
                 const float* word_emb, const float* pos_emb, const float* type_emb,
                 const float* gamma, const float* beta, float eps, int32_t H, void* out,
                 void* stream);
int drt_linear_bf16(const void* X, const void* W, const float* bias, const void* residual,
                    void* Y, int64_t M, int64_t N, int64_t K, int32_t flags, void* stream);
size_t drt_linear_workspace(int64_t M, int64_t N, int64_t K);
int drt_linear_bf16_ws(const void* X, const void* W, const float* bias, const void* residual,
                       void* Y, int64_t M, int64_t N, int64_t K, int32_t flags, void* ws,
                       size_t ws_bytes, void* stream);
int drt_linear_ln_bf16_ws(const void* X, const void* W, const float* bias, const void* residual,
                          const float* gamma, const float* beta, float eps, void* presum, void* out,
                          int64_t M, int64_t N, int64_t K, void* ws, size_t ws_bytes, void* stream);
size_t drt_linear_dgelu_bias_workspace(int64_t M, int64_t N, int64_t K);
int drt_linear_dgelu_bias_bf16(const void* dY, const void* Wt, const void* gelu_pre, void* dX, int64_t M,
                               int64_t N, int64_t K, float* dbias, void* ws, size_t ws_bytes, void* stream);
int drt_linear_bf16_ex(const void* X, const void* W, const float* bias, const void* residual,
                       const void* gelu_pre, void* Y, void* Y_pre, int64_t M, int64_t N, int64_t K,
                       int32_t flags, float drop_p, uint64_t seed, uint64_t site, void* ws,
                       size_t ws_bytes, void* stream);
int drt_layernorm_f32_bf16(const float* X, int64_t M, int32_t H, const float* gamma,
                           const float* beta, float eps, void* out, void* stream);
int drt_layernorm_bf16(const void* X, int64_t M, int32_t H, const float* gamma,
                       const float* beta, float eps, void* out, void* stream);
int drt_attention_bf16(const void* qkv, const int64_t* mask, void* ctx, int64_t B, int64_t L,
                       int32_t heads, int32_t head_dim, float scale, void* stream);
int drt_attention_fwd_lse_bf16(const void* qkv, const int64_t* mask, void* ctx, float* lse, int64_t B,
                               int64_t L, int32_t heads, int32_t head_dim, float scale, void* stream);

size_t drt_layernorm_bwd_workspace(int64_t M, int32_t H);
int drt_layernorm_bwd_bf16(const void* dy, const void* x, const float* gamma, float eps, int64_t M,
                           int32_t H, const void* dres, void* dx, float* dgamma, float* dbeta,
                           void* ws, size_t ws_bytes, void* stream);
int drt_layernorm_bwd_drop_bf16(const void* dy, const void* x, const float* gamma, float eps,
                                int64_t M, int32_t H, const void* dres, void* dx, void* dx_drop,
                                float drop_p, uint64_t seed, uint64_t site, float* dgamma,
                                float* dbeta, void* ws, size_t ws_bytes, void* stream);
int drt_layernorm_bwd_sum_bf16(const void* dy, const void* x, const float* gamma, float eps,
                               int64_t M, int32_t H, const void* dres, void* dx, void* dx_drop,
                               float drop_p, uint64_t seed, uint64_t site, float* dgamma,
                               float* dbeta, float* dsum, void* ws, size_t ws_bytes, void* stream);
size_t drt_colsum_workspace(int64_t M, int64_t N);
int drt_colsum_bf16(const void* x, int64_t M, int64_t N, float* out, void* ws, size_t ws_bytes,
                    void* stream);
int drt_colsum_f32(const float* x, int64_t M, int64_t N, float* out, void* ws, size_t ws_bytes,
                   void* stream);
int drt_gelu_bwd_bf16(const void* dy, const void* pre, int64_t n, void* dx, void* stream);
int drt_transpose_bf16(const void* x, int64_t R, int64_t C, void* y, void* stream);
int drt_transpose_bf16_ld(const void* x, int64_t R, int64_t C, void* y, int64_t ldy, void* stream);
size_t drt_linear_wgrad_workspace(int64_t T, int64_t N, int64_t K);
int drt_linear_wgrad_bf16(const void* dY, const void* X, float* dW, int64_t T, int64_t N, int64_t K, void* ws,
                          size_t ws_bytes, void* stream);
int drt_embed_ln_pre(const int64_t* ids, const int64_t* type_ids, int64_t B, int64_t L,
                     const float* word_emb, const float* pos_emb, const float* type_emb,
                     const float* gamma, const float* beta, float eps, int32_t H, void* out, void* pre,
                     void* stream);
int drt_gelu_bf16(const void* x, int64_t n, void* y, void* stream);
int drt_embedding_bwd(const int64_t* ids, const int64_t* type_ids, const void* d, int64_t B, int64_t L,
                      int32_t H, int64_t padding_idx, float* dword, float* dpos, float* dtype,
                      void* stream);
int drt_embedding_bwd_types(const int64_t* ids, const int64_t* type_ids, int32_t ntypes, const void* d,
// ... 71 lines not shown
```

Before: 82340.

## Add staged threshold-tightening filter scan with strided sample and multi-pass spans

Adds a staged filter pipeline for single-GPU chunked search. A strided sample scan sets an initial per-query threshold, a small first slice of interleaved tile passes tightens it, and the remaining tiles are scanned as one wide span using the tighter threshold. The scan kernels gain a pass-span walker so one launch can cover several interleaved passes. This aims to cut candidate hits and selection work compared with the per-chunk filter-passes path, at the cost of more launches, extra rank-estimation logic and a risk of threshold miscalibration.

```diff
diff --git a/denseretrievaltoolkits_amd/_native.py b/denseretrievaltoolkits_amd/_native.py
--- a/denseretrievaltoolkits_amd/_native.py
+++ b/denseretrievaltoolkits_amd/_native.py
@@ -42,6 +42,11 @@
     ("drt_ip_topk_filter_passes_workspace", c_sz, [c_i64, c_i64, c_i64, c_i32, c_i32]),
     ("drt_ip_topk_filter_passes", c_i32, [c_vp, c_i64, c_vp, c_i64, c_i64, c_i32, c_i32, c_i64, c_vp, c_vp,
                                           c_i32, c_i32, c_vp, c_vp, c_vp, c_sz, c_vp]),
+    ("drt_ip_topk_stage_rank", c_i32, [c_i64, c_i32, c_i32, c_i32]),
+    ("drt_ip_topk_filter_stages_plan", c_i32, [c_i64, c_i64, c_i32, c_i32, c_vp]),
+    ("drt_ip_topk_filter_stages_workspace", c_sz, [c_i64, c_i64, c_i64, c_i32, c_i32, c_i32]),
+    ("drt_ip_topk_filter_stages", c_i32, [c_vp, c_i64, c_vp, c_i64, c_i64, c_i32, c_i32, c_i64, c_i32, c_vp, c_vp,
+                                          c_i32, c_vp, c_vp, c_vp, c_sz, c_vp]),
     ("drt_ip_topk_dist_filter_lists", c_i32, [c_vp, c_i64, c_vp, c_i64, c_i64, c_i32, c_i32, c_i64, c_vp, c_i32,
                                               c_vp, c_vp, c_vp, c_sz, c_vp]),
     ("drt_ip_topk_dist_filter_lists_at", c_i32, [c_vp, c_i64, c_vp, c_i64, c_i64, c_i32, c_i32, c_i64, c_vp,
diff --git a/denseretrievaltoolkits_amd/csrc/search.hip b/denseretrievaltoolkits_amd/csrc/search.hip
--- a/denseretrievaltoolkits_amd/csrc/search.hip
+++ b/denseretrievaltoolkits_amd/csrc/search.hip
@@ -8,9 +8,19 @@
 constexpr int kHitCap = 1024;
 constexpr int kTopRL = 4;
 
-__host__ __device__ __forceinline__ int pass_tiles(int ntiles, int npass, int pass) {
-  return npass <= 1 ? ntiles : (pass < ntiles ? (ntiles - 1 - pass) / npass + 1 : 0);
-}
+__host__ __device__ __forceinline__ int pass_tiles(int ntiles, int npass, int pass, int span = 1) {
+  if (npass <= 1) return ntiles;
+  const int over = ntiles % npass - pass;
+  return ntiles / npass * span + (over < 0 ? 0 : over < span ? over : span);
+}
+
+struct PassWalk {
+  int first, dt;
+  __device__ __forceinline__ void init(int t0, int tstep, int tmul, int tph, int span) {
+    first = t0 / span * tmul + tph + t0 % span;
+    dt = tstep / span * tmul;
+  }
+};
 
 __device__ __forceinline__ void glds16(const void* gsrc, uint32_t lds_addr) {
   uint32_t keep;
@@ -491,17 +501,22 @@
   const int64_t qbase = (int64_t)blockIdx.y * kQueriesPerWG;
   const int tmul = a.npass > 1 ? a.npass : 1;
   const int tph = a.npass > 1 ? a.pass : 0;
+  const int span = a.npass > 1 && a.pspan > 1 ? a.pspan : 1;
   const int tall = (int)((a.nrows + kT16 - 1) / kT16);
-  const int ntiles = pass_tiles(tall, a.npass, a.pass);
+  const int ntiles = pass_tiles(tall, a.npass, a.pass, span);
   const uint32_t nrows = (uint32_t)a.nrows;
   const int t0 = blockIdx.x;
   const int tstep = gridDim.x;
   const int my_tiles = t0 < ntiles ? (ntiles - 1 - t0) / tstep + 1 : 0;
   if (my_tiles == 0) return;
-  const int partial_tile = ((a.nrows & (kT16 - 1)) != 0 && (tall - 1) % tmul == tph) ? ntiles - 1 : -1;
+  const int partial_tile = (a.nrows & (kT16 - 1)) != 0 ? tall - 1 : -1;
   const uint32_t ring = lds_addr_of(smem);
-  const int64_t tile_stride = (int64_t)tstep * tmul * kT16 * a.ldp * 2;
-  const char* next_base = (const char*)(a.P + ((int64_t)t0 * tmul + tph) * kT16 * a.ldp);
+  PassWalk pw;
+  pw.init(t0, tstep, tmul, tph, span);
+  int nxt = pw.first, cur = pw.first;
+  const int64_t tile_bytes = (int64_t)kT16 * a.ldp * 2;
+  const int64_t tile_stride = pw.dt * tile_bytes;
+  const char* next_base = (const char*)a.P + nxt * tile_bytes;
 
   const int64_t qw = qbase + wave * 16;
   const int64_t qg = qw + r;
@@ -529,10 +544,9 @@
 #pragma unroll
   for (int p = 0; p < PD; ++p) {
     if (p < my_tiles) {
-      const int tile = t0 + p * tstep;
-      lt.template issue<NT>(a, ring + p * C::TILE_BYTES, next_base, tile == partial_tile, tile * tmul + tph, wave,
-                            lane);
+      lt.template issue<NT>(a, ring + p * C::TILE_BYTES, next_base, nxt == partial_tile, nxt, wave, lane);
       next_base += tile_stride;
+      nxt += pw.dt;
     }
   }
   if (wave >= NW / 2) __builtin_amdgcn_s_setprio(1);
@@ -613,7 +627,6 @@
   uint32_t rbA = 0, rbB = 0;
   int buf = 0;
   auto iter = [&](int it, f32x4& acc, uint32_t& rb, const f32x4& prev, uint32_t rb_prev) {
-    const int tile = t0 + it * tstep;
     if (it + PD <= my_tiles) {
       wait_vmcnt<C::GLDS_PER_WAVE * (PD - 2)>();
     } else if (it + 1 < my_tiles) {
@@ -621,15 +634,15 @@
     }
     lds_barrier();
     if (it + PD < my_tiles) {
-      const int ntile = tile + PD * tstep;
-      lt.template issue<NT>(a, ring + buf * C::TILE_BYTES, next_base, ntile == partial_tile, ntile * tmul + tph,
-                            wave, lane);
+      lt.template issue<NT>(a, ring + buf * C::TILE_BYTES, next_base, nxt == partial_tile, nxt, wave, lane);
       next_base += tile_stride;
+      nxt += pw.dt;
     }
     const int nslot = buf + 1 == C::NBUF ? 0 : buf + 1;
     mma_roll(acc, nslot);
     if (it > 0) epilogue(prev, rb_prev);
-    rb = (uint32_t)(tile * tmul + tph) * kT16 + 4 * kq;
+    rb = (uint32_t)cur * kT16 + 4 * kq;
+    cur += pw.dt;
     buf = nslot;
   };
   for (int it = 0; it < my_tiles; it += 2) {
@@ -679,17 +692,22 @@
   const int64_t qbase = (int64_t)blockIdx.y * kQueriesPerWG32;
   const int tmul = a.npass > 1 ? a.npass : 1;
   const int tph = a.npass > 1 ? a.pass : 0;
+  const int span = a.npass > 1 && a.pspan > 1 ? a.pspan : 1;
   const int tall = (int)((a.nrows + kT16 - 1) / kT16);
-  const int ntiles = pass_tiles(tall, a.npass, a.pass);
+  const int ntiles = pass_tiles(tall, a.npass, a.pass, span);
   const uint32_t nrows = (uint32_t)a.nrows;
   const int t0 = blockIdx.x;
   const int tstep = gridDim.x;
   const int my_tiles = t0 < ntiles ? (ntiles - 1 - t0) / tstep + 1 : 0;
   if (my_tiles == 0) return;
-  const int partial_tile = ((a.nrows & (kT16 - 1)) != 0 && (tall - 1) % tmul == tph) ? ntiles - 1 : -1;
+  const int partial_tile = (a.nrows & (kT16 - 1)) != 0 ? tall - 1 : -1;
   const uint32_t ring = lds_addr_of(smem);
-  const int64_t tile_stride = (int64_t)tstep * tmul * kT16 * a.ldp * 2;
-  const char* next_base = (const char*)(a.P + ((int64_t)t0 * tmul + tph) * kT16 * a.ldp);
+  PassWalk pw;
+  pw.init(t0, tstep, tmul, tph, span);
+  int nxt = pw.first, cur = pw.first;
+  const int64_t tile_bytes = (int64_t)kT16 * a.ldp * 2;
+  const int64_t tile_stride = pw.dt * tile_bytes;
+  const char* next_base = (const char*)a.P + nxt * tile_bytes;
 
   const int64_t qw = qbase + wave * 32;
   bf16x8 qf0[KS], qf1[KS];
@@ -725,10 +743,9 @@
 #pragma unroll
   for (int p = 0; p < PD; ++p) {
     if (p < my_tiles) {
-      const int tile = t0 + p * tstep;
-      lt.template issue<false>(a, ring + p * C::TILE_BYTES, next_base, tile == partial_tile, tile * tmul + tph, wave,
-                               lane);
+      lt.template issue<false>(a, ring + p * C::TILE_BYTES, next_base, nxt == partial_tile, nxt, wave, lane);
       next_base += tile_stride;
+      nxt += pw.dt;
     }
   }
   if (wave >= NW / 2) __builtin_amdgcn_s_setprio(1);
@@ -781,7 +798,6 @@
   int buf = 0;
   auto iter = [&](int it, f32x4& acc0, f32x4& acc1, uint32_t& rb, const f32x4& prev0, const f32x4& prev1,
                   uint32_t rb_prev) {
-    const int tile = t0 + it * tstep;
     if (it + PD <= my_tiles) {
       wait_vmcnt<C::GLDS_PER_WAVE * (PD - 2)>();
     } else if (it + 1 < my_tiles) {
@@ -789,7 +805,6 @@
     }
     lds_barrier();
     const bool do_dma = it + PD < my_tiles;
-    const int ntile = tile + PD * tstep;
     const int pslot = buf == 0 ? NB - 1 : buf - 1;
     const int nslot = buf + 1 == NB ? 0 : buf + 1;
     acc0 = (f32x4){0.f, 0.f, 0.f, 0.f};
@@ -801,14 +816,15 @@
       af[s % RD] = s + RD < KS ? frag(buf, s + RD) : frag(nslot, s + RD - KS);
       __builtin_amdgcn_sched_barrier(0);
       if (s == KS / 4 && do_dma) {
-        lt.template issue<false>(a, ring + pslot * C::TILE_BYTES, next_base, ntile == partial_tile,
-                                 ntile * tmul + tph, wave, lane);
+        lt.template issue<false>(a, ring + pslot * C::TILE_BYTES, next_base, nxt == partial_tile, nxt, wave, lane);
         next_base += tile_stride;
+        nxt += pw.dt;
       }
       __builtin_amdgcn_sched_barrier(0);
     }
     if (it > 0) epilogue(prev0, prev1, rb_prev);
-    rb = (uint32_t)(tile * tmul + tph) * kT16 + 4 * kq;
+    rb = (uint32_t)cur * kT16 + 4 * kq;
+    cur += pw.dt;
     buf = nslot;
   };
   f32x4 a0, a1, b0, b1;
@@ -956,12 +972,14 @@
 static int launch_scan_d(const ScanArgs& a, int mode, hipStream_t s) {
   if (a.nq == 0 || a.nrows == 0) return DRT_OK;
   constexpr bool kLean = D <= 768;
+  const int span = a.pspan > 1 ? a.pspan : 1;
   if (a.npass > 1 && (mode != SCAN_FILTER || !kLean || a.row0 != 0 || a.rstride != 1 || a.pass < 0 ||
-                      a.pass >= a.npass))
+                      a.pass + span > a.npass))
     return DRT_EINVAL;
-  const int64_t ntiles = pass_tiles((int)((a.nrows + kT16 - 1) / kT16), a.npass, a.pass);
+  const int64_t ntiles = pass_tiles((int)((a.nrows + kT16 - 1) / kT16), a.npass, a.pass, span);
   if (ntiles == 0) return DRT_OK;
-  const dim3 grid = scan16_grid(a.nq, ntiles * kT16);
+  auto span_grid = [span](dim3 g) { return dim3((g.x + span - 1) / span * span, g.y); };
+  const dim3 grid = span_grid(scan16_grid(a.nq, ntiles * kT16));
   const unsigned gy = grid.y;
   if (mode == SCAN_FILTER) {
     const double eh = a.exp_hits > 0 ? (double)a.exp_hits : (double)a.cap / 4.0;
@@ -971,7 +989,7 @@
       lean = a.row0 == 0 && a.rstride == 1;
       if (lean) {
         if (gy > 1) {
-          const dim3 grid32 = scan16_grid(a.nq, ntiles * kT16, kQueriesPerWG32);
+          const dim3 grid32 = span_grid(scan16_grid(a.nq, ntiles * kT16, kQueriesPerWG32));
           hipLaunchKernelGGL((ip_scan32r_kernel<D>), grid32, dim3(512), 0, s, a);
         } else {
           hipLaunchKernelGGL((ip_scan16r_kernel<D, true>), grid, dim3(512), 0, s, a);
@@ -1429,9 +1447,14 @@
 }
 
 int32_t drt_ip_topk_tighten_rank(int64_t n_local, int32_t npasses, int32_t k) {
-  if (n_local <= 0 || npasses <= 1 || k < 1) return 0;
+  return drt_ip_topk_stage_rank(n_local, npasses, 1, k);
+}
+
+int32_t drt_ip_topk_stage_rank(int64_t n_local, int32_t npass, int32_t span, int32_t k) {
+  if (n_local <= 0 || npass <= 1 || span < 1 || span >= npass || k < 1) return 0;
   const int64_t tall = (n_local + kT16 - 1) / kT16;
-  const int64_t t0 = (tall + npasses - 1) / npasses;
+  if (tall > 0x7FFFFFFF) return 0;
+  const int64_t t0 = pass_tiles((int)tall, npass, 0, span);
   if (t0 >= tall) return 0;
   const double C = (double)tall / (double)t0;
   for (int64_t r = 1; r < ((int64_t)1 << 24); ++r) {
@@ -1478,13 +1501,153 @@
       if ((rc = launch_scan(a, d, SCAN_FILTER, f.s, PROF_SCAN))) return rc;
       if (tighten && ps == 0) {
         const ProfPair pp = prof_begin(PROF_SELECT, f.s);
-        launch_tighten(nq, (const uint64_t*)f.scan.out, f.p.cap, f.cnt, tau, (int)r, tau1, pass0, f.s);
+        launch_tighten(nq, (const uint64_t*)f.scan.out, f.p.cap, f.cnt, tau, tau, (int)r, tau1, pass0, f.s);
         prof_end(pp, f.s);
         DRT_CHECK_HIP(hipGetLastError());
       }
     }
   }
   f.sel.pass0 = tighten ? pass0 : nullptr;
+  return filter_select(f);
+}
+
+constexpr int kStageB = 8;
+constexpr int kStageAHits = 4;
+
+struct StagePlan {
+  bool staged;
+  int32_t npass;
+  int32_t r_a, r_b, r_c;
+  int64_t m, stride;
+};
+
+static StagePlan make_stage_plan(const TopkPlan& p, int32_t nch) {
+  StagePlan sp{};
+  const int64_t n = p.n, tall = (n + kT16 - 1) / kT16;
+  if (!p.sample || nch < 2 || nch > 128 || tall > 0x7FFFFFFF) return sp;
+  sp.npass = kStageB * nch;
+  const int64_t ta = pass_tiles((int)tall, sp.npass, 0, 1);
+  if (ta == 0 || pass_tiles((int)tall, sp.npass, kStageB, sp.npass - kStageB) == 0) return sp;
+  sp.r_b = drt_ip_topk_stage_rank(n, sp.npass, 1, (int32_t)p.k);
+  sp.r_c = drt_ip_topk_stage_rank(n, sp.npass, kStageB, (int32_t)p.k);
+  if (sp.r_b <= 0 || sp.r_c <= 0) return sp;
+  int64_t r = 12, m = 0;
+  for (int it = 0; it < 8; ++it) {
+    m = std::min<int64_t>(n, std::max<int64_t>(2 * r, ta * kT16 * r / ((int64_t)kStageAHits * sp.r_b)));
+    int64_t r2 = 1;
+    while (poisson_tail_ge((double)p.k * (double)m / (double)n, r2) > 1e-9 && r2 < 100000) ++r2;
+    if (r2 == r) break;
+    r = r2;
+  }
+  sp.r_a = (int32_t)r;
+  sp.stride = std::max<int64_t>(1, n / m);
+  sp.m = (n - sp.stride / 2 + sp.stride - 1) / sp.stride;
+  sp.staged = sp.m >= r;
+  return sp;
+}
+
+static size_t stages_plan_bytes(int64_t nq, int64_t n_local, int64_t n_global, int32_t k, int32_t k_sample) {
+  return std::max(make_dist_plan(nq, n_local, n_global, k).total,
+                  make_dist_plan(nq, n_local, n_global, k_sample).total);
+}
+
+size_t drt_ip_topk_filter_stages_workspace(int64_t nq, int64_t n_local, int64_t n_global, int32_t d, int32_t k,
+                                           int32_t k_sample) {
+  if (!valid_dist_dims(nq, n_local, n_global, d, k) || k_sample < 1 || k_sample > k) return 0;
+  const TopkPlan p = make_dist_plan(nq, n_local, n_global, k);
+  return stages_layout(stages_plan_bytes(nq, n_local, n_global, k, k_sample), p.nq_pad,
+                       drt_ip_topk_sample_rank(k_sample)).total;
+}
+
+int32_t drt_ip_topk_filter_stages_plan(int64_t nq, int64_t n, int32_t k, int32_t nch, int64_t* out) {
+  if (!valid_dist_dims(nq, n, n, 64, k) || !out) return DRT_EINVAL;
+  const StagePlan sp = make_stage_plan(make_dist_plan(nq, n, n, k), nch);
+  const int64_t v[6] = {sp.staged, sp.npass, sp.m, sp.r_a, sp.r_b, sp.r_c};
+  std::copy(v, v + 6, out);
+  return DRT_OK;
+}
+
+int drt_ip_topk_filter_stages(const void* Q, int64_t nq, const void* P, int64_t n_local, int64_t n_global, int32_t d,
+                              int32_t k, int64_t id_offset, int32_t k_sample, const float* tau, uint64_t* packed,
+                              int32_t nch, float* taus_out, uint32_t* state_out, void* ws, size_t ws_bytes,
+                              void* stream) {
+  DRT_REQUIRE(d <= 768 && n_local < ((int64_t)1 << 32) && nch >= 1 && nch <= 128);
+  DRT_REQUIRE(k_sample >= 1 && k_sample <= k);
+  DRT_REQUIRE(tau != nullptr || (n_local == n_global && id_offset == 0));
+  FilterRun f;
+  int rc = filter_setup(f, Q, nq, P, n_local, n_global, d, k, id_offset, tau ? (const void*)tau : Q, packed, ws,
+                        ws_bytes, stream);
+  if (rc || nq == 0) return rc;
+  const int32_t r_s = drt_ip_topk_sample_rank(k_sample);
+  const StagesLayout sl = stages_layout(stages_plan_bytes(nq, n_local, n_global, k, k_sample), f.p.nq_pad, r_s);
+  DRT_REQUIRE(ws_bytes >= sl.total);
+  const int64_t ts = taus_out ? nq : f.p.nq_pad;
+  float* T = taus_out ? taus_out : (float*)(f.w + sl.off_taus);
+  uint32_t* st = state_out ? state_out : (uint32_t*)(f.w + sl.off_state);
+  uint32_t* st1 = st + nq * 4;
+  StagePlan sp = make_stage_plan(f.p, nch);
+  const int64_t nlists = sp.staged ? 4 * (int64_t)scan16_grid(nq, sp.m).x : 0;
+  if (sp.staged && !tau && !(nlists * kTopRL <= kKthChunk && nlists * kTopRL <= (int64_t)align_up(f.p.m, 4)))
+    sp.staged = false;
+
+  if (!sp.staged || n_local == 0) {
+    if (!tau) {
+      uint32_t* best = (uint32_t*)(f.w + sl.off_best);
+      if ((rc = drt_ip_topk_dist_sample(Q, nq, P, n_local, n_global, d, k_sample, best, ws, ws_bytes, stream)))
+        return rc;
+      if ((rc = drt_ip_topk_dist_tau(best, nq, 1, k_sample, T, stream))) return rc;
+    } else {
+      DRT_CHECK_HIP(hipMemcpyAsync(T, tau, (size_t)nq * 4, hipMemcpyDeviceToDevice, f.s));
+    }
+    if ((rc = drt_ip_topk_filter_passes(Q, nq, P, n_local, n_global, d, k, id_offset, T, packed, nch, -1, T + ts, st,
+                                        ws, ws_bytes, stream)))
+      return rc;
+    DRT_CHECK_HIP(hipMemcpyAsync(T + 2 * ts, T + ts, (size_t)nq * 4, hipMemcpyDeviceToDevice, f.s));
+    DRT_CHECK_HIP(hipMemcpyAsync(st1, st, (size_t)nq * 16, hipMemcpyDeviceToDevice, f.s));
+    return DRT_OK;
+  }
+
+  if ((rc = filter_begin(f, tau != nullptr))) return rc;
+  if (tau) {
+    DRT_CHECK_HIP(hipMemcpyAsync(T, tau, (size_t)nq * 4, hipMemcpyDeviceToDevice, f.s));
+  } else {
+    ScanArgs a = scan_args(Q, nq, P, d);
+    a.row0 = sp.stride / 2;
+    a.nrows = sp.m;
+    a.rstride = sp.stride;
+    a.out = f.w + f.p.off_sample;
+    a.cap = nlists * kTopRL;
+    DRT_CHECK_HIP(hipMemsetAsync(a.out, 0xFF, (size_t)nq * a.cap * 4, f.s));
+    if ((rc = launch_scan(a, d, SCAN_TOPR, f.s, PROF_SAMPLE))) return rc;
+    const ProfPair pp = prof_begin(PROF_SELECT, f.s);
+    launch_kth_final(nq, (const uint32_t*)a.out, (int)nlists, sp.r_a, (int64_t)kTopRL, (int64_t)a.cap, T, nullptr,
+                     f.cnt, kTopRL, f.s);
+    prof_end(pp, f.s);
+    DRT_CHECK_HIP(hipGetLastError());
+  }
+  auto scan = [&](int pass, int span, const float* thr) {
+    ScanArgs a = f.scan;
+    a.npass = sp.npass;
+    a.pass = pass;
+    a.pspan = span;
+    a.tau = thr;
+    a.exp_hits = 1;
+    return launch_scan(a, d, SCAN_FILTER, f.s, PROF_SCAN);
+  };
+  auto tighten = [&](const float* prev, int r, float* next, uint32_t* state) {
+    const ProfPair pp = prof_begin(PROF_SELECT, f.s);
+    launch_tighten(nq, (const uint64_t*)f.scan.out, f.p.cap, f.cnt, prev, T, r, next, state, f.s);
+    prof_end(pp, f.s);
+    return hip_status(hipGetLastError());
+  };
+  if ((rc = scan(0, 1, T))) return rc;
+  if ((rc = tighten(T, sp.r_b, T + ts, st))) return rc;
+  for (int ps = 1; ps < kStageB; ps *= 2)
+    if ((rc = scan(ps, ps, T + ts))) return rc;
+  if ((rc = tighten(T + ts, sp.r_c, T + 2 * ts, st1))) return rc;
+  for (int g = 1; g < nch; ++g)
+    if ((rc = scan(kStageB * g, kStageB, T + 2 * ts))) return rc;
+  f.sel.pass0 = st1;
   return filter_select(f);
 }
 
diff --git a/denseretrievaltoolkits_amd/csrc/search_internal.h b/denseretrievaltoolkits_amd/csrc/search_internal.h
--- a/denseretrievaltoolkits_amd/csrc/search_internal.h
+++ b/denseretrievaltoolkits_amd/csrc/search_internal.h
@@ -50,7 +50,8 @@
                                    int64_t qstride, float* tau, uint32_t* best, uint32_t* zero, int len,
                                    hipStream_t s);
 DRT_INTERNAL void launch_tighten(int64_t nq, const uint64_t* keys, int64_t cap, const uint32_t* counts,
-                                 const float* tau0, int r, float* tau1, uint32_t* pass0, hipStream_t s);
+                                 const float* tau_prev, const float* tau_base, int r, float* tau1, uint32_t* pass0,
+                                 hipStream_t s);
 
 enum { SCAN_FILTER = 0, SCAN_DENSE = 1, SCAN_TOPR = 2 };
 
@@ -71,6 +72,7 @@
   uint32_t row_base;
   int32_t npass;
   int32_t pass;
+  int32_t pspan;
 };
 
 static inline ScanArgs scan_args(const void* Q, int64_t nq, const void* P, int32_t d) {
@@ -176,6 +178,19 @@
   return l;
 }
 
+struct StagesLayout {
+  size_t off_state, off_taus, off_best, total;
+};
+static inline StagesLayout stages_layout(size_t plan_total, int64_t nq_pad, int64_t best_keys) {
+  WsBump b{passes_layout(plan_total, nq_pad).total};
+  StagesLayout l;
+  l.off_state = b.take((size_t)nq_pad * 32);
+  l.off_taus = b.take((size_t)nq_pad * 12);
+  l.off_best = b.take((size_t)nq_pad * best_keys * 4);
+  l.total = b.o;
+  return l;
+}
+
 static inline int64_t resolve_width(int64_t n) { return align_up(std::max<int64_t>(n, 4), 4); }
 
 struct ResolveLayout {
diff --git a/denseretrievaltoolkits_amd/csrc/select.hip b/denseretrievaltoolkits_amd/csrc/select.hip
--- a/denseretrievaltoolkits_amd/csrc/select.hip
+++ b/denseretrievaltoolkits_amd/csrc/select.hip
@@ -482,16 +482,18 @@
 constexpr int kTightThreads = 256;
 
 __global__ __launch_bounds__(kTightThreads) void tighten_kernel(const uint64_t* keys, int64_t cap,
-                                                                const uint32_t* counts, const float* tau0, int r,
-                                                                float* tau1, uint32_t* pass0) {
+                                                                const uint32_t* counts, const float* tau_prev,
+                                                                const float* tau_base, int r, float* tau1,
+                                                                uint32_t* pass0) {
   __shared__ uint32_t hist[256];
   __shared__ uint32_t sh_prefix, sh_rem;
   __shared__ uint32_t red[kTightThreads / 64];
   const int tid = threadIdx.x;
   const int64_t q = blockIdx.x;
   const uint32_t c = counts[q * kCntStride];
-  const float t0 = tau0[q];
-  if (!((int64_t)c <= cap && c >= (uint32_t)r && t0 == t0)) {
+  const float t0 = tau_prev[q];
+  const float tb = tau_base[q];
+  if (!((int64_t)c <= cap && t0 == t0)) {
     if (tid == 0) {
       tau1[q] = t0;
       pass0[q * 4 + 0] = c;
@@ -503,7 +505,7 @@
   }
   const uint64_t* kq = keys + q * cap;
   uint32_t prefix = 0, mask = 0, rem = (uint32_t)r;
-  for (int shift = 24; shift >= 0; shift -= 8) {
+  for (int shift = 24; shift >= 0 && c >= (uint32_t)r; shift -= 8) {
     hist[tid] = 0;
     __syncthreads();
     for (uint32_t j = tid; j < c; j += kTightThreads) {
@@ -539,7 +541,11 @@
     rem = sh_rem;
     mask |= 255u << shift;
   }
-  const float t1 = desc_key_to_score(prefix);
+  float t1 = t0;
+  if (c >= (uint32_t)r) {
+    const float tr = desc_key_to_score(prefix);
+    t1 = tr > t0 ? tr : t0;
+  }
   uint32_t n = 0;
   for (uint32_t j = tid; j < c; j += kTightThreads) n += key_score(kq[j]) >= t1 ? 1u : 0u;
 #pragma unroll
@@ -552,7 +558,7 @@
     tau1[q] = t1;
     pass0[q * 4 + 0] = c;
     pass0[q * 4 + 1] = tot;
-    pass0[q * 4 + 2] = t1 > t0 ? 1u : 0u;
+    pass0[q * 4 + 2] = t1 > tb ? 1u : 0u;
     pass0[q * 4 + 3] = 0;
   }
 }
@@ -916,10 +922,10 @@
                      tau, best, zero, len);
 }
 
-void launch_tighten(int64_t nq, const uint64_t* keys, int64_t cap, const uint32_t* counts, const float* tau0, int r,
-                    float* tau1, uint32_t* pass0, hipStream_t s) {
-  hipLaunchKernelGGL(tighten_kernel, dim3((unsigned)nq), dim3(kTightThreads), 0, s, keys, cap, counts, tau0, r, tau1,
-                     pass0);
-}
-
-}
+void launch_tighten(int64_t nq, const uint64_t* keys, int64_t cap, const uint32_t* counts, const float* tau_prev,
+                    const float* tau_base, int r, float* tau1, uint32_t* pass0, hipStream_t s) {
+  hipLaunchKernelGGL(tighten_kernel, dim3((unsigned)nq), dim3(kTightThreads), 0, s, keys, cap, counts, tau_prev,
+                     tau_base, r, tau1, pass0);
+}
+
+}
diff --git a/denseretrievaltoolkits_amd/csrc/torch_ops.cpp b/denseretrievaltoolkits_amd/csrc/torch_ops.cpp
--- a/denseretrievaltoolkits_amd/csrc/torch_ops.cpp
+++ b/denseretrievaltoolkits_amd/csrc/torch_ops.cpp
@@ -408,6 +408,47 @@
          (uint64_t*)packed.data_ptr<int64_t>(), (int32_t)npasses, (int32_t)r,
          tau1.has_value() ? tau1->data_ptr<float>() : nullptr,
          pass0.has_value() ? (uint32_t*)pass0->data_ptr<int32_t>() : nullptr);
+}
+
+void filter_stages_into(const Tensor& q_, const Tensor& p_, int64_t n_global, int64_t k, int64_t id_offset,
+                        int64_t k_sample, const c10::optional<Tensor>& tau_, int64_t nch, Tensor& packed, Tensor& taus,
+                        const c10::optional<Tensor>& state) {
+  need(q_, "q", at::kBFloat16, 2);
+  need(p_, "p", at::kBFloat16, 2);
+  need(packed, "packed", at::kLong, 2);
+  need(taus, "taus", at::kFloat, 2);
+  const c10::DeviceGuard g(q_.device());
+  const Tensor q = q_.contiguous(), p = p_.contiguous();
+  const int64_t nq = q.size(0);
+  TORCH_CHECK_VALUE(q.size(1) <= 768, "the staged filter takes d <= 768");
+  TORCH_CHECK_VALUE(nch >= 1 && nch <= 128, "nch must be in [1, 128]");
+  TORCH_CHECK_VALUE(packed.is_contiguous() && packed.size(0) == nq && packed.size(1) == k + 1,
+                    "packed must be a contiguous [nq, k + 1] tensor");
+  TORCH_CHECK_VALUE(taus.is_contiguous() && taus.size(0) == 3 && taus.size(1) == nq,
+                    "taus must be a contiguous [3, nq] tensor");
+  Tensor tau;
+  if (tau_.has_value()) {
+    need(*tau_, "tau", at::kFloat, 1);
+    tau = tau_->contiguous();
+    TORCH_CHECK_VALUE(tau.size(0) == nq, "tau must hold one threshold per query");
+  }
+  if (state.has_value()) {
+    need(*state, "state", at::kInt, 3);
+    TORCH_CHECK_VALUE(state->is_contiguous() && state->size(0) == 2 && state->size(1) == nq && state->size(2) == 4,
+                      "state must be a contiguous [2, nq, 4] tensor");
+  }
+  const size_t wsb = drt_ip_topk_filter_stages_workspace(nq, p.size(0), n_global, (int32_t)q.size(1), (int32_t)k,
+                                                         (int32_t)k_sample);
+  TORCH_CHECK_VALUE(wsb > 0 || nq == 0, "unsupported staged filter shape nq=", nq, " n_local=", p.size(0),
+                    " n_global=", n_global, " d=", q.size(1), " k=", k, " k_sample=", k_sample);
+  Tensor ws = workspace(q, wsb);
+  check_rc(drt_ip_topk_filter_stages(q.data_ptr(), nq, p.size(0) ? p.data_ptr() : nullptr, p.size(0), n_global,
+                                     (int32_t)q.size(1), (int32_t)k, id_offset, (int32_t)k_sample,
+                                     tau.defined() ? tau.data_ptr<float>() : nullptr,
+                                     (uint64_t*)packed.data_ptr<int64_t>(), (int32_t)nch, taus.data_ptr<float>(),
+                                     state.has_value() ? (uint32_t*)state->data_ptr<int32_t>() : nullptr,
+                                     ws.data_ptr(), wsb, stream_of(q)),
+           "drt_ip_topk_filter_stages");
 }
 
 void filter_lists_into(const Tensor& q_, const Tensor& p_, int64_t n_global, int64_t k, int64_t id_offset,
@@ -762,6 +803,8 @@
         "Tensor(a!) packed) -> ()");
   m.def("filter_passes_into(Tensor q, Tensor p, int n_global, int k, int id_offset, Tensor tau, int npasses, int r, "
         "Tensor(a!) packed, Tensor(b!)? tau1=None, Tensor(c!)? pass0=None) -> ()");
+  m.def("filter_stages_into(Tensor q, Tensor p, int n_global, int k, int id_offset, int k_sample, Tensor? tau, int nch, "
+        "Tensor(a!) packed, Tensor(b!) taus, Tensor(c!)? state=None) -> ()");
   m.def("merge_packed(Tensor parts, int k, int n_global, int k_cert=-1) -> (Tensor, Tensor, Tensor)");
   m.def("topk_exclude(Tensor scores, Tensor ids, Tensor excl, Tensor excl_off, Tensor? ceiling, int skip, int k_out) -> "
         "(Tensor, Tensor, Tensor)");
@@ -787,6 +830,7 @@
   m.impl("ip_topk.out", &ip_topk_out);
   m.impl("dist_filter_chunks_into", &dist_filter_chunks_into);
   m.impl("filter_passes_into", &filter_passes_into);
+  m.impl("filter_stages_into", &filter_stages_into);
   m.impl("ip_topk_resolve", &ip_topk_resolve);
   m.impl("ip_topk_resolve_wide", &ip_topk_resolve_wide);
   m.impl("ip_topk_large", &ip_topk_large);
diff --git a/denseretrievaltoolkits_amd/kernels.py b/denseretrievaltoolkits_amd/kernels.py
--- a/denseretrievaltoolkits_amd/kernels.py
+++ b/denseretrievaltoolkits_amd/kernels.py
@@ -278,6 +278,28 @@
     ops.load().filter_passes_into(q, p, n_global, k, id_offset, tau, npasses, r, packed, tau1, pass0)
 
 
+def stage_rank(n_local: int, npass: int, span: int, k: int) -> int:
+    return int(_native.load().drt_ip_topk_stage_rank(n_local, npass, span, k))
+
+
+def filter_stages_plan(nq: int, n: int, k: int, nch: int) -> dict:
+    import ctypes
+    out = (ctypes.c_int64 * 6)()
+    if _native.load().drt_ip_topk_filter_stages_plan(nq, n, k, nch, out) != 0:
+        raise ValueError(f"unsupported staged filter shape nq={nq} n={n} k={k}")
+    return dict(zip(("staged", "npass", "m", "r_a", "r_b", "r_c"), (int(v) for v in out)))
+
+
+def filter_stages_into(q: torch.Tensor, p: torch.Tensor, n_global: int, k: int, id_offset: int, nch: int,
+                       packed: torch.Tensor, k_sample: Optional[int] = None, tau: Optional[torch.Tensor] = None,
+                       state: Optional[torch.Tensor] = None) -> torch.Tensor:
+    _require_device(q, p, packed)
+    taus = torch.empty((3, q.shape[0]), dtype=torch.float32, device=q.device)
+    ops.load().filter_stages_into(q, p, n_global, k, id_offset, k if k_sample is None else k_sample, tau, nch,
+                                  packed, taus, state)
+    return taus
+
+
 def dist_filter_lists_into(q: torch.Tensor, p: torch.Tensor, n_global: int, k: int, id_offset: int,
                            lists: torch.Tensor, q0: int, packed: torch.Tensor) -> None:
     _require_device(q, p, lists, packed)
diff --git a/denseretrievaltoolkits_amd/ops.py b/denseretrievaltoolkits_amd/ops.py
--- a/denseretrievaltoolkits_amd/ops.py
+++ b/denseretrievaltoolkits_amd/ops.py
@@ -116,6 +116,10 @@
     def _(q, p, n_global, k, id_offset, tau, npasses, r, packed, tau1=None, pass0=None):
         return None
 
+    @lib.register_fake("drt::filter_stages_into")
+    def _(q, p, n_global, k, id_offset, k_sample, tau, nch, packed, taus, state=None):
+        return None
+
     @lib.register_fake("drt::dist_filter_lists_into")
     def _(q, p, n_global, k, id_offset, lists, q0, packed):
         return None
diff --git a/denseretrievaltoolkits_amd/search.py b/denseretrievaltoolkits_amd/search.py
--- a/denseretrievaltoolkits_amd/search.py
+++ b/denseretrievaltoolkits_amd/search.py
@@ -76,6 +76,7 @@
 GROUP_MIN_ROWS = 500_000
 GROUP_CHUNK_ROWS = 1_250_000
 TIGHTEN_AFTER_FIRST_PASS = True
+STAGED_MIN_ROWS = 1_000_000
 
 
 def group_chunks(nrows: int, chunk_rows: int = None, nch: int = None):
@@ -109,7 +110,9 @@
         return
     kc = kernels.refine_width(k)
     nq = GROUP_QUERIES
-    ws = int(_native.load().drt_ip_topk_dist_workspace(nq, local.ntotal, n_global, local.dp, kc))
+    lib = _native.load()
+    ws = max(int(lib.drt_ip_topk_dist_workspace(nq, local.ntotal, n_global, local.dp, kc)),
+             int(lib.drt_ip_topk_filter_stages_workspace(nq, local.ntotal, n_global, local.dp, kc, k)))
     nparts = max(1, len(chunks or [0]))
     lists = nq * (kc + 1) * 8 * (nparts + 1)
     outs = nq * kc * (4 + 8 + 4) + nq * k * (4 + 8) * 2
@@ -138,14 +141,20 @@
                         side: _SideChannel = None):
     sizes = [q.shape[0] for q in qs]
     qg = qs[0] if len(qs) == 1 else torch.cat(qs)
-    best = local.dist_sample(qg, n_global, k)
-    lists = gather(best).contiguous()
-    tau = kernels.dist_tau(lists, k)
+    chunked = chunks is not None and len(chunks) > 1 and qg.shape[1] <= 768
+    one_gpu = TIGHTEN_AFTER_FIRST_PASS and world == 1 and offset == 0 and n_global == local.rows.shape[0]
+    staged = chunked and one_gpu and n_global >= STAGED_MIN_ROWS
+    if not staged:
+        best = local.dist_sample(qg, n_global, k)
+        lists = gather(best).contiguous()
+        tau = kernels.dist_tau(lists, k)
     kc = kernels.refine_width(k) if stats is not None else k
     lc = kernels.exchange_cap(kc, world) if world > 1 and getattr(local, "exchange_capped", True) else kc
-    if chunks is not None and len(chunks) > 1 and qg.shape[1] <= 768:
+    if chunked:
         lists = torch.empty((qg.shape[0], lc + 1), dtype=torch.int64, device=qg.device)
-        if TIGHTEN_AFTER_FIRST_PASS and world == 1 and offset == 0 and n_global == local.rows.shape[0]:
+        if staged:
+            tau = kernels.filter_stages_into(qg, local.rows, n_global, lc, offset, len(chunks), lists, k_sample=k)[2]
+        elif one_gpu:
             kernels.filter_passes_into(qg, local.rows, n_global, lc, offset, tau, len(chunks), lists)
         else:
             starts = [a for a, _ in chunks] + [chunks[-1][1]]
diff --git a/include/drt.h b/include/drt.h
--- a/include/drt.h
+++ b/include/drt.h
@@ -101,6 +101,15 @@
                               int64_t n_global, int32_t d, int32_t k, int64_t id_offset,
                               const float* tau, uint64_t* packed, int32_t npasses, int32_t r,
                               float* tau1_out, uint32_t* pass0_out, void* ws, size_t ws_bytes,
+                              void* stream);
+int32_t drt_ip_topk_stage_rank(int64_t n_local, int32_t npass, int32_t span, int32_t k);
+int32_t drt_ip_topk_filter_stages_plan(int64_t nq, int64_t n, int32_t k, int32_t nch, int64_t* out);
+size_t drt_ip_topk_filter_stages_workspace(int64_t nq, int64_t n_local, int64_t n_global, int32_t d,
+                                           int32_t k, int32_t k_sample);
+int drt_ip_topk_filter_stages(const void* Q, int64_t nq, const void* P, int64_t n_local,
+                              int64_t n_global, int32_t d, int32_t k, int64_t id_offset,
+                              int32_t k_sample, const float* tau, uint64_t* packed, int32_t nch,
+                              float* taus_out, uint32_t* state_out, void* ws, size_t ws_bytes,
                               void* stream);
 int drt_ip_topk_dist_filter_lists(const void* Q, int64_t nq, const void* P, int64_t n_local,
                                   int64_t n_global, int32_t d, int32_t k, int64_t id_offset,
```

Result: no change. 82590, median of 6 (+0.3%).
